# BurryChen/lv_slam

Measured on AMD Instinct MI355X. Metric: NDT registrations/sec (64k-pt Velodyne pairs), higher is better.
Workload: dtype f32 terms, f64 accumulation

## Files before the change

### include/mi355_ndt.h

```cpp
#ifndef MI355_NDT_H_
#define MI355_NDT_H_

#include <stddef.h>
#include <stdint.h>

#ifdef __cplusplus
extern "C" {
#endif

#define MI355NDT_OK               0
#define MI355NDT_ERR_BAD_HANDLE  (-1)
#define MI355NDT_ERR_BAD_ARG     (-2)
#define MI355NDT_ERR_HIP         (-3)
#define MI355NDT_ERR_GRID        (-4)
#define MI355NDT_ERR_NO_DEVICE   (-5)
#define MI355NDT_ERR_UNSUPPORTED (-6)
#define MI355NDT_WARN_TOLERANCE_ARITH 1
#define MI355NDT_TOLERANCE_MIN_HITS   4096
#define MI355NDT_ERR_STATE       (-7)

enum mi355ndt_neighbor { MI355NDT_KDTREE = 0, MI355NDT_DIRECT26 = 1, MI355NDT_DIRECT7 = 2, MI355NDT_DIRECT1 = 3 };
enum mi355ndt_variant { MI355NDT_VARIANT_OMP = 0 , MI355NDT_VARIANT_PCA = 1  };

typedef struct mi355ndt_params {
  float  resolution;
  double step_size;
  double outlier_ratio;
  double trans_epsilon;
  int    max_iterations;
  int    neighbor_mode;
  int    variant;
  int    min_points_per_voxel;
  double min_covar_eigvalue_mult;
} mi355ndt_params;

typedef struct mi355ndt_result {
  float     final_colmajor[16];
  double    trans_probability;
  double    score;
  int       iterations;
  int       converged;
  int       sweeps;
  int       status;
  long long hits_last;
} mi355ndt_result;

typedef struct mi355ndt_voxel {
  int32_t idx;
  int32_t n;
  double  mean[3];
  float   icov[9];
  int32_t weight;
} mi355ndt_voxel;

typedef struct mi355ndt_profile {
  double    sweep_ms;
  long long sweep_launches;
  double    sweep_alg_bytes;
  long long sweep_hits;
  long long sweep_points;
  double    build_ms;
  long long build_launches;
  double    build_alg_bytes;
  double    update_ms;
  long long update_launches;
  long long async_fallbacks;
  long long stream_launches;
  long long stream_carried;
  long long stream_redone;
  long long cloud_uploads;
  long long cloud_upload_bytes;
  long long cloud_transfers;
  long long cloud_promotions;
  long long stream_reserved_slots;
  long long stream_launch_slots;
} mi355ndt_profile;

typedef struct mi355ndt_handle mi355ndt_handle;

const char* mi355ndt_version(void);
int mi355ndt_device_count(void);
int mi355ndt_host_numa_node(int device);

int mi355ndt_default_params(mi355ndt_params* p);

int mi355ndt_create(const mi355ndt_params* params, int device, mi355ndt_handle** out);
int mi355ndt_destroy(mi355ndt_handle* h);

int mi355ndt_set_params(mi355ndt_handle* h, const mi355ndt_params* params);
int mi355ndt_get_params(const mi355ndt_handle* h, mi355ndt_params* out);

int mi355ndt_set_stream(mi355ndt_handle* h, void* hip_stream);
const char* mi355ndt_last_error(const mi355ndt_handle* h);


int mi355ndt_set_target(mi355ndt_handle* h, const void* pts, size_t n, size_t stride_bytes);
int mi355ndt_set_source(mi355ndt_handle* h, const void* pts, size_t n, size_t stride_bytes);
int mi355ndt_promote_source_to_target(mi355ndt_handle* h);
int mi355ndt_align(mi355ndt_handle* h, const float guess_colmajor[16], mi355ndt_result* out);
int mi355ndt_get_aligned(mi355ndt_handle* h, void* out_pts, size_t stride_bytes);

int mi355ndt_get_incremental(mi355ndt_handle* h, int pair, float transformation_colmajor[16], float previous_colmajor[16]);

int mi355ndt_get_fitness_score(mi355ndt_handle* h, double max_range, double* score, long long* n_inliers);
int mi355ndt_fitness_score_T(mi355ndt_handle* h, const float T_colmajor[16], double max_range, double* score, long long* n_inliers);

int mi355ndt_calculate_score(mi355ndt_handle* h, const void* pts, size_t n, size_t stride_bytes, double* score);

int mi355ndt_convert_transform(const double x[6], float out_colmajor[16]);

enum mi355ndt_option {
  MI355NDT_OPT_F32_SUM_ORDER = 1,
  MI355NDT_OPT_ASYNC_ALIGN = 2,
  MI355NDT_OPT_DEBUG_ASYNC_ABORT = 3,
  MI355NDT_OPT_STREAM_THRESHOLD = 4,
  MI355NDT_OPT_STREAM_RESERVE = 5,
  MI355NDT_OPT_DEBUG_ASYNC_RINGS = 6,
  MI355NDT_OPT_ARITH = 7
};
int mi355ndt_set_option(mi355ndt_handle* h, int option, int value);
int mi355ndt_get_option(const mi355ndt_handle* h, int option, int* value);

int mi355ndt_derivatives(mi355ndt_handle* h, const double p[6], double* score, double g[6], double H[36], long long* hits);
int mi355ndt_compute_hessian(mi355ndt_handle* h, const double p[6], double H[36]);
int mi355ndt_derivatives_T(mi355ndt_handle* h, const float T_colmajor[16], const float Rj_rowmajor[9],
                           double* score, double g[6], double H[36], long long* hits);
int mi355ndt_get_grid(mi355ndt_handle* h, int pair, int min_b[3], int max_b[3], int div_b[3], int* n_voxels);
int mi355ndt_get_voxels(mi355ndt_handle* h, int pair, mi355ndt_voxel* out, size_t capacity);


int mi355ndt_batch_reserve(mi355ndt_handle* h, int n_pairs, size_t max_target_pts, size_t max_source_pts);
int mi355ndt_batch_set_target(mi355ndt_handle* h, int pair, const void* pts, size_t n, size_t stride_bytes);
int mi355ndt_batch_set_source(mi355ndt_handle* h, int pair, const void* pts, size_t n, size_t stride_bytes);
int mi355ndt_batch_set_clouds(mi355ndt_handle* h, int first_pair, int n, const void* const* targets, const size_t* target_counts,
                              const void* const* sources, const size_t* source_counts, size_t stride_bytes, int n_threads);
int mi355ndt_batch_bind_device(mi355ndt_handle* h, int n_pairs,
                               const float* d_targets, const int* target_counts, size_t target_pitch,
                               const float* d_sources, const int* source_counts, size_t source_pitch);
int mi355ndt_batch_build_targets(mi355ndt_handle* h);
int mi355ndt_batch_align(mi355ndt_handle* h, const float* guesses_colmajor, mi355ndt_result* out);
int mi355ndt_batch_size(const mi355ndt_handle* h);
int mi355ndt_batch_fitness_scores(mi355ndt_handle* h, const float* T_colmajor, double max_range, double* scores, long long* n_inliers);
int mi355ndt_batch_pose_records(mi355ndt_handle* h, int id_base, int id_stride, void* d_records, size_t capacity);

int mi355ndt_stream_begin(mi355ndt_handle* h, int n_contexts , int max_pairs, size_t max_target_pts, size_t max_source_pts);
int mi355ndt_stream_submit(mi355ndt_handle* h, int n_pairs, const float* d_targets, const int* target_counts, size_t target_pitch,
                           const float* d_sources, const int* source_counts, size_t source_pitch, const float* guesses_colmajor,
                           long long* batch_id);
int mi355ndt_stream_submit_host(mi355ndt_handle* h, int n_pairs, const void* const* targets, const size_t* target_counts, const void* const* sources,
                                const size_t* source_counts, size_t stride_bytes, const float* guesses_colmajor, int n_threads, long long* batch_id);
int mi355ndt_stream_collect(mi355ndt_handle* h, long long batch_id, mi355ndt_result* out);
int mi355ndt_stream_pose_records(mi355ndt_handle* h, void* d_records, size_t capacity, int id_base, int id_stride);
int mi355ndt_pack_pose_records(const mi355ndt_result* results, int n, int id_base, int id_stride, void* records, size_t capacity);
int mi355ndt_stream_end(mi355ndt_handle* h);

int mi355ndt_set_latency_mode(mi355ndt_handle* h, int on);

typedef struct mi355ndt_seq_params {
  double keyframe_delta_trans;
  double keyframe_delta_angle;
  double keyframe_delta_time;
} mi355ndt_seq_params;

typedef struct mi355ndt_seq_frame {
  double odom_colmajor[16];
  float  tf_s2k_colmajor[16];
  double trans_probability;
  double dx, da, dt;
  int    key_id;
  int    new_keyframe;
  int    iterations, converged;
// ... 31 lines not shown
```

### lv_slam_amd/csrc/mi355_ndt.hip

```cpp
#include <hip/hip_runtime.h>

#include <cstdio>
#include <cstdlib>
#include <cstddef>
#include <cstring>
#include <string>
#include <vector>
#include <algorithm>
#include <cmath>
#include <mutex>
#include <atomic>
#include <thread>
#include <sched.h>
#include <fstream>
#include <chrono>

#include "mi355_ndt.h"
#include "ndt_math.hpp"
#include "ndt_types.hpp"
#include "ndt_build.hpp"
#include "ndt_segsort.hpp"
#include "ndt_sweep.hpp"
#include "ndt_update.hpp"
#include "ndt_hessian.hpp"
// ... 16 lines not shown
  int device = 0;
  hipStream_t stream = nullptr;
  bool own_stream = true;
  mi355ndt_params prm;
  std::string err;

  int n_pairs = 0, cap_pairs = 0;
  size_t tgt_pitch = 0, src_pitch = 0;
  size_t own_tgt_pitch = 0, own_src_pitch = 0;
  int own_tgt_pairs = 0, own_src_pairs = 0;
  float *d_tgt_own = nullptr, *d_src_own = nullptr;
  const float *d_tgt = nullptr, *d_src = nullptr;
  int *d_tgt_cnt = nullptr, *d_src_cnt = nullptr;
  std::vector<int> h_tgt_cnt, h_src_cnt;
  std::vector<int> up_tgt_cnt, up_src_cnt;
  bool targets_built = false, have_target = false, have_source = false;
  bool aligned_once = false;
  bool icov64_built = false;
  bool cent_built = false;
  float grid_resolution = 0.f;

  unsigned* d_minmax = nullptr;
  GridDesc* d_grid = nullptr;
  unsigned *d_nwords = nullptr, *d_word_off = nullptr;
  unsigned *d_keys_a = nullptr, *d_keys_b = nullptr;
  unsigned *d_vals_a = nullptr, *d_vals_b = nullptr;
  size_t keys_cap = 0;
  BitWord* d_words = nullptr; size_t words_cap = 0;
  VoxelRec* d_recs = nullptr; int *d_vox_idx = nullptr, *d_vox_n = nullptr;
  unsigned* d_seg_start = nullptr; double* d_sums = nullptr;
  unsigned *d_heads = nullptr, *d_head_cnt = nullptr; size_t heads_cap = 0, head_cnt_cap = 0;
  float* d_cent = nullptr; double* d_icov64 = nullptr; size_t icov64_cap = 0;
  int* d_kdw = nullptr; size_t kdw_cap = 0; bool kdw_built = false;
  float4* d_sorted = nullptr; size_t sorted_cap = 0; bool leaf_sorted = false;
  unsigned* d_rs_hist = nullptr; unsigned* d_rs_offs = nullptr; size_t rs_cap = 0;
  unsigned *d_cstart = nullptr, *d_cend = nullptr; size_t cell_cap = 0; bool cells_ready = false; int last_cb = 0;
  double* d_fit = nullptr; size_t fit_cap = 0;
  BitWord* d_fwords = nullptr; size_t fwords_cap = 0; unsigned* d_fruns = nullptr; size_t fruns_cap = 0; bool fit_index_ready = false;
  int* d_fit_items = nullptr; size_t fit_items_cap = 0; float* d_fit_T = nullptr; size_t fit_T_cap = 0;
  float *d_pf_in = nullptr, *d_pf_out = nullptr; unsigned char* d_pf_keep = nullptr; unsigned *d_pf_keys = nullptr, *d_pf_vals = nullptr;
  int *d_pf_flag = nullptr, *d_pf_pos = nullptr, *d_pf_mm = nullptr; PfGrid* d_pf_grid = nullptr; void* d_pf_tmp = nullptr;
  size_t pf_cap = 0, pf_tmp_bytes = 0; int pf_count = 0; size_t pf_pitch = 0;
  float last_final[16] = {1,0,0,0, 0,1,0,0, 0,0,1,0, 0,0,0,1};
  size_t recs_per_pair = 0, recs_cap = 0;
  unsigned* h_pin_u = nullptr;

  PairState* d_state = nullptr;
  double* d_partials = nullptr; size_t partials_cap = 0;
  int chunks_per_pair = 0;
  int rows_per_pair = 0, pts_per_chunk = CHUNK_PTS;
  int items_per_pair = 0;
  bool async_force = false;
  bool async_align = true;
  int* d_ring = nullptr; size_t ring_cap_total = 0; unsigned* d_arrived = nullptr; size_t arrived_cap = 0; AsyncCtl* d_actl = nullptr;
  AsyncCtl* h_pin_actl = nullptr;
  AsyncTab* d_atab = nullptr;
  unsigned debug_abort_pos = 0xFFFFFFFFu;
  unsigned debug_ring_mask = 0xFFu;
  int arith = 0;
  VoxelRecF* d_recs_fast = nullptr; size_t recs_fast_cap = 0; bool recs_fast_built = false;
  int f32_sum_order = 0;
  double gauss_last[3] = {0, 0, 0};
  float* d_score_pts = nullptr; size_t score_pts_cap = 0; double* d_score_part = nullptr; size_t score_part_cap = 0;
  bool latency_mode = false;
  bool seq_running = false;
  int fine_it = 0;
  int fine_tiles = 2;
  int* d_grid_of = nullptr; size_t grid_of_cap = 0;
  const int* d_grid_of_use = nullptr;
  SeqState* d_seq = nullptr; mi355ndt_seq_frame* d_seq_out = nullptr; double* d_stamps = nullptr; size_t seq_cap = 0;
  volatile int* h_seq_flags = nullptr; int* d_seq_flags = nullptr;
  float* d_guess = nullptr;
  float* h_pin_guess = nullptr;
  mi355ndt_result* d_results = nullptr;
  int* d_active = nullptr;
  int* d_active_list = nullptr;
  SweepCtl* d_ctl = nullptr;
  int ctl_idx = 0;
  int n_cu = 256;
  int dyn_shift = -1;
  int* h_pin_active = nullptr;
  hipEvent_t ev_burst[2] = {nullptr, nullptr};
  unsigned long long* d_hits = nullptr;
  float* d_hook = nullptr;
  float* d_aligned = nullptr; size_t aligned_cap = 0;
  float* h_pin_aligned = nullptr; size_t pin_aligned_cap = 0;
  struct UpSlot { float* h = nullptr; float* d = nullptr; size_t cap = 0; hipEvent_t ev = nullptr; bool used = false, filling = false; };
  static constexpr int UP_SLOTS = 12;
  UpSlot up[UP_SLOTS];
  int up_next = 0;
  static constexpr int UP_STREAMS = 4;
  hipStream_t copy_stream[UP_STREAMS] = {nullptr, nullptr, nullptr, nullptr};
  hipEvent_t ev_uploads[UP_STREAMS] = {nullptr, nullptr, nullptr, nullptr}, ev_compute = nullptr;
  bool uploads_pending = false;
  std::mutex up_mtx;

  bool async_build = false;
  int plan_cb = 0; size_t plan_words = 0;
  unsigned* d_bstat = nullptr;
  bool counts_preloaded = false;
  bool build_stamped = false;
  bool word_off_cleared = false;
  size_t last_total_words = 0;

  struct StreamCtx {
    mi355ndt_handle* e = nullptr;
// ... 161 lines not shown
  std::ifstream f("/sys/devices/system/node/node" + std::to_string(node) + "/cpulist");
  std::string txt;
  if (!f || !std::getline(f, txt)) return false;
  bool any = false;
  size_t pos = 0;
  while (pos < txt.size()) {
    size_t comma = txt.find(',', pos);
    std::string part = txt.substr(pos, comma == std::string::npos ? std::string::npos : comma - pos);
    size_t dash = part.find('-');
    int lo = atoi(part.c_str()), hi = dash == std::string::npos ? lo : atoi(part.c_str() + dash + 1);
    for (int c = lo; c <= hi && c < CPU_SETSIZE; c++) { CPU_SET(c, set); any = true; }
    if (comma == std::string::npos) break;
    pos = comma + 1;
  }
  return any;
}

int mi355ndt_default_params(mi355ndt_params* p) {
  if (!p) return MI355NDT_ERR_BAD_ARG;
  p->resolution = 1.0f;
  p->step_size = 0.1;
  p->outlier_ratio = 0.55;
  p->trans_epsilon = 0.1;
  p->max_iterations = 35;
  p->neighbor_mode = MI355NDT_DIRECT7;
  p->variant = MI355NDT_VARIANT_OMP;
  p->min_points_per_voxel = 6;
  p->min_covar_eigvalue_mult = 0.01;
  return MI355NDT_OK;
}

int mi355ndt_destroy(mi355ndt_handle* h);

int mi355ndt_create(const mi355ndt_params* params, int device, mi355ndt_handle** out) {
  if (!out) return MI355NDT_ERR_BAD_ARG;
  *out = nullptr;
  int n = 0;
  if (hipGetDeviceCount(&n) != hipSuccess || n <= 0) return MI355NDT_ERR_NO_DEVICE;
  if (device < 0 || device >= n) return MI355NDT_ERR_BAD_ARG;
  mi355ndt_params p;
  mi355ndt_default_params(&p);
  if (params) p = *params;
  int rc = check_params(p);
  if (rc) return rc;
  mi355ndt_handle* h = new mi355ndt_handle();
  h->device = device;
  h->prm = p;
  gauss_constants3(0.55, 1.0f, h->gauss_last);
  { hipDeviceProp_t pr; if (hipGetDeviceProperties(&pr, device) == hipSuccess && pr.multiProcessorCount > 0) h->n_cu = pr.multiProcessorCount; }
  if (const char* e = std::getenv("MI355NDT_LEAF_SORTED")) h->leaf_sorted = std::atoi(e) != 0;
  if (const char* e = std::getenv("MI355NDT_FINE_TILES")) { const int v = std::atoi(e); if (v == 1 || v == 2) h->fine_tiles = v; }
  if (const char* e = std::getenv("MI355NDT_ARITH")) h->arith = std::atoi(e) == 1 ? 1 : 0;
  if (const char* e = std::getenv("MI355NDT_ASYNC")) { h->async_align = std::atoi(e) != 0; h->async_force = std::atoi(e) == 2; }
  if (const char* e = std::getenv("MI355NDT_SWEEP_DYN_SHIFT")) { const int v = std::atoi(e); if (v >= 0 && v <= 30) h->dyn_shift = v; }
  if (hipSetDevice(device) != hipSuccess || hipStreamCreateWithFlags(&h->stream, hipStreamNonBlocking) != hipSuccess) {
    delete h;
    return MI355NDT_ERR_HIP;
  }
  if (hipHostMalloc((void**)&h->h_pin_u, 4 * sizeof(unsigned)) != hipSuccess ||
      hipHostMalloc((void**)&h->h_pin_active, 128 * sizeof(int)) != hipSuccess ||
      hipMalloc((void**)&h->d_active, 128 * sizeof(int)) != hipSuccess ||
      hipMalloc((void**)&h->d_ctl, 2 * sizeof(SweepCtl)) != hipSuccess ||
      hipMalloc((void**)&h->d_hits, sizeof(unsigned long long)) != hipSuccess ||
      hipMalloc((void**)&h->d_hook, 64 * sizeof(double)) != hipSuccess ||
      hipEventCreateWithFlags(&h->ev_compute, hipEventDisableTiming) != hipSuccess ||
      hipEventCreateWithFlags(&h->ev_burst[0], hipEventDisableTiming) != hipSuccess ||
      hipEventCreateWithFlags(&h->ev_burst[1], hipEventDisableTiming) != hipSuccess) {
    mi355ndt_destroy(h);
    return MI355NDT_ERR_HIP;
  }
  for (int i = 0; i < mi355ndt_handle::UP_STREAMS; i++)
    if (hipStreamCreateWithFlags(&h->copy_stream[i], hipStreamNonBlocking) != hipSuccess ||
        hipEventCreateWithFlags(&h->ev_uploads[i], hipEventDisableTiming) != hipSuccess) { mi355ndt_destroy(h); return MI355NDT_ERR_HIP; }
  *out = h;
  return MI355NDT_OK;
}

int mi355ndt_stream_end(mi355ndt_handle* h);
int mi355ndt_destroy(mi355ndt_handle* h) {
  if (!h) return MI355NDT_ERR_BAD_HANDLE;
  (void)hipSetDevice(h->device);
  (void)hipStreamSynchronize(h->stream);
  if (h->stream_on) (void)mi355ndt_stream_end(h);
  void* ptrs[] = {h->d_tgt_own, h->d_src_own, h->d_tgt_cnt, h->d_src_cnt, h->d_grid, h->d_nwords, h->d_word_off,
                  h->d_keys_a, h->d_keys_b, h->d_vals_a, h->d_vals_b, h->d_words, h->d_recs, h->d_vox_idx, h->d_vox_n,
                  h->d_state, h->d_partials, h->d_guess, h->d_results, h->d_active, h->d_hook, h->d_aligned, h->d_hits, h->d_seg_start, h->d_heads, h->d_head_cnt, h->d_sums,
                  h->d_cent, h->d_icov64, h->d_kdw, h->d_rs_hist, h->d_rs_offs, h->d_active_list, h->d_ctl, h->d_cstart, h->d_cend, h->d_fit, h->d_fwords, h->d_fruns, h->d_fit_items, h->d_fit_T, h->d_pf_in, h->d_pf_out, h->d_pf_keep, h->d_pf_keys,
                  h->d_pf_vals, h->d_pf_flag, h->d_pf_pos, h->d_pf_mm, h->d_pf_grid, h->d_pf_tmp, h->d_score_pts, h->d_score_part,
                  h->d_ring, h->d_arrived, h->d_actl, h->d_atab, h->d_sorted, h->d_recs_fast};
  for (void* p : ptrs) if (p) (void)hipFree(p);
  for (void* p : {(void*)h->d_grid_of, (void*)h->d_seq, (void*)h->d_seq_out, (void*)h->d_stamps}) if (p) (void)hipFree(p);
  if (h->h_seq_flags) (void)hipHostFree((void*)h->h_seq_flags);
  for (hipStream_t cs : h->copy_stream) if (cs) (void)hipStreamSynchronize(cs);
  for (auto& u : h->up) { if (u.h) (void)hipHostFree(u.h); if (u.d) (void)hipFree(u.d); if (u.ev) (void)hipEventDestroy(u.ev); }
  if (h->h_pin_aligned) (void)hipHostFree(h->h_pin_aligned);
  for (hipEvent_t e : h->ev_uploads) if (e) (void)hipEventDestroy(e);
  if (h->ev_compute) (void)hipEventDestroy(h->ev_compute);
  for (hipStream_t cs : h->copy_stream) if (cs) (void)hipStreamDestroy(cs);
  if (h->h_pin_actl) (void)hipHostFree(h->h_pin_actl);
  if (h->h_pin_u) (void)hipHostFree(h->h_pin_u);
  if (h->h_pin_active) (void)hipHostFree(h->h_pin_active);
  if (h->h_pin_guess) (void)hipHostFree(h->h_pin_guess);
  for (hipEvent_t e : h->ev_burst) if (e) (void)hipEventDestroy(e);
  for (hipEvent_t e : h->ev_pool) (void)hipEventDestroy(e);
  for (auto* v : {&h->ev_sweep, &h->ev_update, &h->ev_build})
    for (auto& e : *v) { if (!e.first_shared) (void)hipEventDestroy(e.first); (void)hipEventDestroy(e.second); }
  if (h->own_stream && h->stream) (void)hipStreamDestroy(h->stream);
  delete h;
  return MI355NDT_OK;
}

int mi355ndt_get_params(const mi355ndt_handle* h, mi355ndt_params* out) {
  if (!h) return MI355NDT_ERR_BAD_HANDLE;
  if (!out) return MI355NDT_ERR_BAD_ARG;
  *out = h->prm;
  return MI355NDT_OK;
// ... 296 lines not shown
  if (h->ev_last_fresh && h->ev_last) {
    v.push_back({h->ev_last, nullptr, true});
    h->ev_last_fresh = false;
    return hipSuccess;
  }
  hipEvent_t a;
  hipError_t e = ev_take(h, &a); if (e != hipSuccess) return e;
  v.push_back({a, nullptr, false});
  return hipEventRecord(a, h->stream);
}
static hipError_t ev_end(mi355ndt_handle* h, std::vector<mi355ndt_handle::EvSpan>& v) {
  hipEvent_t b;
  hipError_t e = ev_take(h, &b); if (e != hipSuccess) return e;
  v.back().second = b;
  h->ev_last = b;
  h->ev_last_fresh = true;
  return hipEventRecord(b, h->stream);
}
static void ev_collect(mi355ndt_handle* h, std::vector<mi355ndt_handle::EvSpan>& v, double& ms, long long& n) {
  for (auto& e : v) {
    float t = 0;
    if (e.second && hipEventElapsedTime(&t, e.first, e.second) == hipSuccess) { ms += t; n++; }
    if (!e.first_shared) h->ev_pool.push_back(e.first);
    if (e.second) h->ev_pool.push_back(e.second);
  }
  v.clear();
  h->ev_last_fresh = false;
}
int mi355ndt_profile_enable(mi355ndt_handle* h, int on) {
  if (!h) return MI355NDT_ERR_BAD_HANDLE;
  h->prof = on != 0;
  if (h->stream_on) for (int c = 0; c < h->s_nctx; c++) if (h->sctx[c].e) { h->sctx[c].e->ev_pool_target = 128; (void)mi355ndt_profile_enable(h->sctx[c].e, on); }
  if (h->prof) {
    HIPCHK(h, hipSetDevice(h->device));
    while (h->ev_pool.size() < h->ev_pool_target) {
      hipEvent_t e;
      HIPCHK(h, hipEventCreate(&e));
      h->ev_pool.push_back(e);
    }
  }
  return MI355NDT_OK;
}
int mi355ndt_profile_reset(mi355ndt_handle* h) {
  if (!h) return MI355NDT_ERR_BAD_HANDLE;
  (void)hipSetDevice(h->device);
  (void)hipStreamSynchronize(h->stream);
  double d; long long n;
  ev_collect(h, h->ev_sweep, d, n); ev_collect(h, h->ev_update, d, n); ev_collect(h, h->ev_build, d, n);
  if (h->stream_on) for (int c = 0; c < h->s_nctx; c++) if (mi355ndt_handle* e = h->sctx[c].e) {
    ev_collect(e, e->ev_sweep, d, n); ev_collect(e, e->ev_update, d, n); ev_collect(e, e->ev_build, d, n);
    e->P = mi355ndt_profile{};
  }
  h->P = mi355ndt_profile{};
  (void)hipMemsetAsync(h->d_hits, 0, sizeof(unsigned long long), h->stream);
  (void)hipStreamSynchronize(h->stream);
  return MI355NDT_OK;
}
int mi355ndt_profile_get(mi355ndt_handle* h, mi355ndt_profile* out) {
  if (!h) return MI355NDT_ERR_BAD_HANDLE;
  if (!out) return MI355NDT_ERR_BAD_ARG;
  HIPCHK(h, hipSetDevice(h->device));
  HIPCHK(h, hipStreamSynchronize(h->stream));
  ev_collect(h, h->ev_sweep, h->P.sweep_ms, h->P.sweep_launches);
  ev_collect(h, h->ev_update, h->P.update_ms, h->P.update_launches);
  ev_collect(h, h->ev_build, h->P.build_ms, h->P.build_launches);
  if (h->stream_on) for (int c = 0; c < h->s_nctx; c++) if (mi355ndt_handle* e = h->sctx[c].e) {
    ev_collect(e, e->ev_sweep, h->P.sweep_ms, h->P.sweep_launches);
    ev_collect(e, e->ev_update, h->P.update_ms, h->P.update_launches);
    ev_collect(e, e->ev_build, h->P.build_ms, h->P.build_launches);
    h->P.build_alg_bytes += e->P.build_alg_bytes; e->P.build_alg_bytes = 0;
    { std::lock_guard<std::mutex> lk(e->up_mtx);
      h->P.cloud_uploads += e->P.cloud_uploads; e->P.cloud_uploads = 0; h->P.cloud_upload_bytes += e->P.cloud_upload_bytes; e->P.cloud_upload_bytes = 0;
      h->P.cloud_transfers += e->P.cloud_transfers; e->P.cloud_transfers = 0; }
  }
  unsigned long long hh = 0;
  HIPCHK(h, hipMemcpy(&hh, h->d_hits, sizeof hh, hipMemcpyDeviceToHost));
  *out = h->P;
  if (h->stream_on) { out->stream_reserved_slots = h->s_reserve_wg; out->stream_launch_slots = h->s_launch_slots; }
  out->sweep_hits += (long long)hh;
  out->sweep_alg_bytes += 64.0 * (double)hh;
  return MI355NDT_OK;
}

static int build_targets_impl(mi355ndt_handle* h);
int mi355ndt_batch_build_targets(mi355ndt_handle* h) {
  if (!h) return MI355NDT_ERR_BAD_HANDLE;
  NOT_IN_STREAM(h);
  const int rc = build_targets_impl(h);
  if (rc != MI355NDT_OK && h->ev_compute) (void)compute_enqueued(h);
  return rc;
}
static int build_targets_impl(mi355ndt_handle* h) {
  if (h->n_pairs <= 0 || !h->d_tgt) return MI355NDT_ERR_STATE;
  HIPCHK(h, hipSetDevice(h->device));
  { int rcu = uploads_before_compute(h); if (rcu) return rcu; }
  const int B = h->n_pairs;
  const size_t pitch = h->tgt_pitch;
  const size_t total = (size_t)B * pitch;
  hipStream_t s = h->stream;
  if (h->async_build && h->counts_preloaded) {
    h->up_tgt_cnt.clear();
  } else if (h->up_tgt_cnt.size() != (size_t)B || !std::equal(h->up_tgt_cnt.begin(), h->up_tgt_cnt.end(), h->h_tgt_cnt.begin())) {
    HIPCHK(h, hipMemcpyAsync(h->d_tgt_cnt, h->h_tgt_cnt.data(), B * sizeof(int), hipMemcpyHostToDevice, s));
    HIPCHK(h, hipStreamSynchronize(s));
    h->up_tgt_cnt.assign(h->h_tgt_cnt.begin(), h->h_tgt_cnt.begin() + B);
  }

  if (total > h->keys_cap) {
    size_t c1 = h->keys_cap, c2 = h->keys_cap, c3 = h->keys_cap, c4 = h->keys_cap;
    HIPCHK(h, grow(h->d_keys_a, c1, total)); HIPCHK(h, grow(h->d_keys_b, c2, total));
    HIPCHK(h, grow(h->d_vals_a, c3, total)); HIPCHK(h, grow(h->d_vals_b, c4, total));
    h->keys_cap = total;
  }
  const int minpts = h->prm.min_points_per_voxel;
  const size_t rpp = pitch / (size_t)minpts + 1;
  if (rpp > ((size_t)1 << ID_BITS)) { h->err = "target too large: voxel ids would not fit the sweep's queue entries"; return MI355NDT_ERR_BAD_ARG; }
  if ((size_t)B * rpp > h->recs_cap || rpp != h->recs_per_pair) {
    size_t need = (size_t)B * rpp, c1 = 0, c2 = 0, c3 = 0, c4 = 0, c5 = 0;
    if (h->d_recs) { HIPCHK(h, hipFree(h->d_recs)); h->d_recs = nullptr; }
    if (h->d_vox_idx) { HIPCHK(h, hipFree(h->d_vox_idx)); h->d_vox_idx = nullptr; }
    if (h->d_vox_n) { HIPCHK(h, hipFree(h->d_vox_n)); h->d_vox_n = nullptr; }
    if (h->d_seg_start) { HIPCHK(h, hipFree(h->d_seg_start)); h->d_seg_start = nullptr; }
    if (h->d_sums) { HIPCHK(h, hipFree(h->d_sums)); h->d_sums = nullptr; }
    if (h->d_cent) { HIPCHK(h, hipFree(h->d_cent)); h->d_cent = nullptr; }
    HIPCHK(h, grow(h->d_recs, c1, need)); HIPCHK(h, grow(h->d_vox_idx, c2, need)); HIPCHK(h, grow(h->d_vox_n, c3, need));
    HIPCHK(h, grow(h->d_seg_start, c4, need)); HIPCHK(h, grow(h->d_sums, c5, need * 9));
    { size_t c6 = 0; HIPCHK(h, grow(h->d_cent, c6, need * 3)); }
    h->recs_cap = need; h->recs_per_pair = rpp;
  }
  h->ev_last_fresh = false;
  const bool build_events = h->prof && !(h->build_stamped && h->async_build);
  if (build_events) HIPCHK(h, ev_begin(h, h->ev_build));
  const int gx = (int)((pitch + 255) / 256);
// ... 275 lines not shown
  unsigned long long* stamp_end = nullptr;
  int claim_items = 1;
  int reserve_wg = 0;
  hipEvent_t ev_prepared = nullptr;
};
#define NDT_CTX_ARGS(i) L.tab.c[i].src, L.tab.c[i].pitch, L.tab.c[i].st, L.tab.c[i].gd, L.tab.c[i].words, L.tab.c[i].recs, L.tab.c[i].partials, L.tab.c[i].src_cnt, \
                        L.tab.c[i].arrived, L.tab.c[i].cent
template <bool PCA, int K, int ORD>
static int launch_async_t(mi355ndt_handle* h, const SweepConst& sc, const AsyncLaunch& L) {
  auto kern = k_align_async<PCA, K, ORD>;
  static std::atomic<int> per_cu_of_device[64];
  int per_cu = per_cu_of_device[h->device & 63].load(std::memory_order_relaxed);
  if (per_cu == 0) {
    if (hipOccupancyMaxActiveBlocksPerMultiprocessor(&per_cu, kern, SWEEP_THREADS, 0) != hipSuccess) { (void)hipGetLastError(); return MI355NDT_ERR_UNSUPPORTED; }
    per_cu_of_device[h->device & 63].store(per_cu, std::memory_order_relaxed);
  }
  const int wpe = sweep_wpe(PCA, K, ORD == 2);
  if (per_cu < wpe || h->n_cu * wpe < 8) return MI355NDT_ERR_UNSUPPORTED;
  dim3 grid((unsigned)std::max(8, h->n_cu * wpe - L.reserve_wg));
  kern<<<grid, SWEEP_THREADS, 0, h->stream>>>(L.tab_dev, L.items_per_pair, L.ring, L.ring_cap, L.ctl, sc, h->prof ? h->d_hits : nullptr,
                                             h->prm.step_size, h->prm.trans_epsilon, h->prm.max_iterations, L.stop_thresh, L.debug_abort_pos, L.debug_ring_mask, L.claim_items,
                                             NDT_CTX_ARGS(0), NDT_CTX_ARGS(1), NDT_CTX_ARGS(2), NDT_CTX_ARGS(3));
  return MI355NDT_OK;
}
template <bool PCA, int K>
static int launch_async_o(mi355ndt_handle* h, const SweepConst& sc, const AsyncLaunch& L) {
  if constexpr (K == 1 || K == 7) { if (sweep_ord(h, sc) == 2) return launch_async_t<PCA, K, 2>(h, sc, L); }
  return h->f32_sum_order == 1 ? launch_async_t<PCA, K, 1>(h, sc, L) : launch_async_t<PCA, K, 0>(h, sc, L);
}
static int launch_async(mi355ndt_handle* h, const SweepConst& sc, const AsyncLaunch& L) {
  hipStream_t s = h->stream;
  {
    const size_t n = std::max(std::max(std::max((size_t)8 * L.ring_cap, (size_t)L.n_new * ASYNC_ARR_STRIDE), sizeof(AsyncCtl) / sizeof(unsigned)), (size_t)L.pose_cap);
    k_async_prepare<<<(unsigned)((n + 255) / 256), 256, 0, s>>>(L.tab, L.tab_dev, L.new_ci, L.n_new, L.st_new, L.guess_new, L.src_cnt_new, L.gd_new, L.arrived_new,
                                                               L.active_list, L.sweep_ctl, L.ring, L.ring_cap, L.ctl, L.prev, L.done_new, L.pose_new, L.pose_cap, L.stamp_end);
    if (L.ev_prepared) HIPCHK(h, hipEventRecord(L.ev_prepared, s));
  }
  if (h->prof) HIPCHK(h, ev_begin(h, h->ev_sweep));
  int rc;
  if (sc.pca) rc = sc.K == 1 ? launch_async_o<true, 1>(h, sc, L) : sc.K == 7 ? launch_async_o<true, 7>(h, sc, L) : launch_async_o<true, 26>(h, sc, L);
  else rc = sc.K == 1 ? launch_async_o<false, 1>(h, sc, L) : sc.K == 7 ? launch_async_o<false, 7>(h, sc, L)
          : sc.K == 26 ? launch_async_o<false, 26>(h, sc, L) : launch_async_o<false, 27>(h, sc, L);
  if (h->prof) HIPCHK(h, ev_end(h, h->ev_sweep));
  return rc;
}
static int async_ring_cap(const mi355ndt_handle* h, long long pairs) {
  const long long cap = (pairs * ((long long)h->prm.max_iterations + 4) + 7) / 8 + 1;
  return cap > (1LL << 26) ? 0 : (int)cap;
}
static void fill_async_ctx(const mi355ndt_handle* e, AsyncCtx& c) {
  SweepConst sc;
  make_sweep_const(e, sc);
  c.src = e->d_src; c.pitch = e->src_pitch; c.st = e->d_state; c.gd = e->d_grid; c.words = e->d_words; c.recs = sweep_recs(e, sc); c.cent = e->d_cent;
  c.partials = e->d_partials; c.src_cnt = e->d_src_cnt; c.arrived = e->d_arrived; c.results = e->d_results; c.n_done = nullptr; c.must_finish = 1; c.pose = nullptr; c.pose_base = 0; c.pose_stride = 0; c.pad_ = 0;
}
extern "C" {
static int align_async(mi355ndt_handle* h, const SweepConst& sc, int B, mi355ndt_result* out) {
  hipStream_t s = h->stream;
  const int ring_cap = async_ring_cap(h, B);
  if (ring_cap == 0) return MI355NDT_ERR_UNSUPPORTED;
  if (grow(h->d_ring, h->ring_cap_total, (size_t)8 * ring_cap) != hipSuccess) { (void)hipGetLastError(); return MI355NDT_ERR_UNSUPPORTED; }
  HIPCHK(h, grow(h->d_arrived, h->arrived_cap, (size_t)B * ASYNC_ARR_STRIDE));
  if (!h->d_actl) HIPCHK(h, hipMalloc((void**)&h->d_actl, sizeof(AsyncCtl)));
  if (!h->d_atab) HIPCHK(h, hipMalloc((void**)&h->d_atab, sizeof(AsyncTab)));
  if (!h->h_pin_actl) HIPCHK(h, hipHostMalloc((void**)&h->h_pin_actl, sizeof(AsyncCtl)));
  AsyncLaunch L;
  memset(&L.tab, 0, sizeof L.tab);
  fill_async_ctx(h, L.tab.c[0]);
  L.new_ci = 0; L.n_new = B;
  L.st_new = h->d_state; L.guess_new = h->d_guess; L.src_cnt_new = h->d_src_cnt; L.gd_new = h->d_grid; L.arrived_new = h->d_arrived;
  L.active_list = h->d_active_list; L.sweep_ctl = h->d_ctl;
  L.tab_dev = h->d_atab; L.ring = h->d_ring; L.ring_cap = ring_cap; L.ctl = h->d_actl; L.prev = nullptr;
  L.items_per_pair = h->items_per_pair; L.stop_thresh = 0; L.debug_abort_pos = h->debug_abort_pos; L.debug_ring_mask = h->debug_ring_mask;
  int rc = launch_async(h, sc, L);
  if (rc) return rc;
  HIPCHK(h, hipMemcpyAsync(h->h_pin_actl, h->d_actl, 8 * sizeof(unsigned), hipMemcpyDeviceToHost, s));
  HIPCHK(h, hipMemcpyAsync(out, h->d_results, (size_t)B * sizeof(mi355ndt_result), hipMemcpyDeviceToHost, s));
  HIPCHK(h, hipStreamSynchronize(s));
  HIPCHK(h, hipGetLastError());
  if (h->h_pin_actl->abort_ || h->h_pin_actl->fin != (unsigned)B) {
    h->P.async_fallbacks++;
    return MI355NDT_ERR_UNSUPPORTED;
  }
  if (h->prof) {
    for (int b = 0; b < B; b++) {
      h->P.sweep_alg_bytes += (double)out[b].sweeps * h->h_src_cnt[b] * (12.0 + 4.0 * sc.K);
      h->P.sweep_points += (long long)out[b].sweeps * h->h_src_cnt[b];
    }
  }
  return MI355NDT_OK;
}

static int batch_align_impl(mi355ndt_handle* h, const float* guesses, mi355ndt_result* out) {
  if (!guesses || !out) return MI355NDT_ERR_BAD_ARG;
  if (h->n_pairs <= 0 || !h->d_tgt || !h->d_src) return MI355NDT_ERR_STATE;
  HIPCHK(h, hipSetDevice(h->device));
  { int rcu = uploads_before_compute(h); if (rcu) return rcu; }
  const bool mt_live = mt_is_live(h->prm);
  const bool pca_kd = h->prm.neighbor_mode == MI355NDT_KDTREE && h->prm.variant == MI355NDT_VARIANT_PCA;
  if (!h->targets_built || (mt_live && !h->icov64_built) || (pca_kd && !h->kdw_built) || (fast_served(h) && !h->recs_fast_built)) { int rc = mi355ndt_batch_build_targets(h); if (rc) return rc; }
  int rc = prep_align_ws(h);
  if (rc) return rc;
  const int B = h->n_pairs;
  hipStream_t s = h->stream;
  SweepConst sc;
  make_sweep_const(h, sc);
  gauss_constants3(h->prm.outlier_ratio, h->prm.resolution, h->gauss_last);
// ... 543 lines not shown
  int rc = upload_cloud(h, h->d_score_pts, pitch, 0, pts, n, stride);
  if (rc) return rc;
  rc = uploads_before_compute(h);
  if (rc) return rc;
  SweepConst sc;
  make_sweep_const(h, sc);
  hipStream_t s = h->stream;
  k_calc_score<<<blocks, SCORE_THREADS, 0, s>>>(h->d_score_pts, pitch, (int)n, h->d_grid, h->d_words, h->d_recs, h->d_icov64, h->d_cent,
                                                h->gauss_last[0], h->gauss_last[1], h->gauss_last[2], sc.kd_r2, sc.leaf_pow2, sc.inv_leaf, h->d_score_part);
  std::vector<double> part((size_t)blocks);
  HIPCHK(h, hipMemcpyAsync(part.data(), h->d_score_part, part.size() * sizeof(double), hipMemcpyDeviceToHost, s));
  HIPCHK(h, hipStreamSynchronize(s));
  HIPCHK(h, hipGetLastError());
  double sum = 0;
  for (int b = 0; b < blocks; b++) sum += part[(size_t)b];
  *score = sum / (double)n;
  return compute_enqueued(h);
}

static void aa_matrix(float angle, int axis, float R[9]) {
  const float ax[3] = {axis == 0 ? 1.f : 0.f, axis == 1 ? 1.f : 0.f, axis == 2 ? 1.f : 0.f};
  const float sn = sinf(angle), c = cosf(angle);
  const float sa[3] = {sn * ax[0], sn * ax[1], sn * ax[2]};
  const float c1[3] = {(1.f - c) * ax[0], (1.f - c) * ax[1], (1.f - c) * ax[2]};
  float tmp = c1[0] * ax[1];
  R[0 * 3 + 1] = tmp - sa[2]; R[1 * 3 + 0] = tmp + sa[2];
  tmp = c1[0] * ax[2];
  R[0 * 3 + 2] = tmp + sa[1]; R[2 * 3 + 0] = tmp - sa[1];
  tmp = c1[1] * ax[2];
  R[1 * 3 + 2] = tmp - sa[0]; R[2 * 3 + 1] = tmp + sa[0];
  for (int a = 0; a < 3; a++) R[a * 3 + a] = c1[a] * ax[a] + c;
}
static void mul33(const float A[9], const float B[9], float C[9]) {
  for (int r = 0; r < 3; r++)
    for (int c = 0; c < 3; c++) C[r * 3 + c] = A[r * 3 + 0] * B[0 * 3 + c] + (A[r * 3 + 1] * B[1 * 3 + c] + A[r * 3 + 2] * B[2 * 3 + c]);
}
int mi355ndt_convert_transform(const double x[6], float out[16]) {
  if (!x || !out) return MI355NDT_ERR_BAD_ARG;
  float Rx[9], Ry[9], Rz[9], A[9], L[9];
  aa_matrix((float)x[3], 0, Rx); aa_matrix((float)x[4], 1, Ry); aa_matrix((float)x[5], 2, Rz);
  mul33(Rx, Ry, A);
  mul33(A, Rz, L);
  for (int r = 0; r < 3; r++) {
    for (int c = 0; c < 3; c++) out[c * 4 + r] = L[r * 3 + c];
    out[12 + r] = (float)x[r];
    out[r * 4 + 3] = 0.f;
  }
  out[15] = 1.f;
  return MI355NDT_OK;
}

int mi355ndt_set_option(mi355ndt_handle* h, int option, int value) {
  if (!h) return MI355NDT_ERR_BAD_HANDLE;
  if (h->stream_on && (option == MI355NDT_OPT_F32_SUM_ORDER || option == MI355NDT_OPT_ARITH || option == MI355NDT_OPT_ASYNC_ALIGN)) NOT_IN_STREAM(h);
  if (option == MI355NDT_OPT_F32_SUM_ORDER) {
    if (value != 0 && value != 1) return MI355NDT_ERR_BAD_ARG;
    h->f32_sum_order = value;
    return MI355NDT_OK;
  }
  if (option == MI355NDT_OPT_ARITH) {
    if (value != 0 && value != 1) return MI355NDT_ERR_BAD_ARG;
    h->arith = value;
    return MI355NDT_OK;
  }
  if (option == MI355NDT_OPT_ASYNC_ALIGN) {
    if (value < 0 || value > 2) return MI355NDT_ERR_BAD_ARG;
    h->async_align = value != 0;
    h->async_force = value == 2;
    return MI355NDT_OK;
  }
  if (option == MI355NDT_OPT_DEBUG_ASYNC_ABORT) {
    h->debug_abort_pos = value < 0 ? 0xFFFFFFFFu : (unsigned)value;
    return MI355NDT_OK;
  }
  if (option == MI355NDT_OPT_DEBUG_ASYNC_RINGS) {
    if ((value & 0xFF) == 0) return MI355NDT_ERR_BAD_ARG;
    h->debug_ring_mask = (unsigned)value & 0xFFu;
    return MI355NDT_OK;
  }
  if (option == MI355NDT_OPT_STREAM_THRESHOLD) {
    if (value < -1 || value > ASYNC_MAX_CARRY) return MI355NDT_ERR_BAD_ARG;
    h->s_thresh_opt = value;
    return MI355NDT_OK;
  }
  if (option == MI355NDT_OPT_STREAM_RESERVE) {
    if (value < -1 || value > 4096) return MI355NDT_ERR_BAD_ARG;
    h->s_reserve_opt = value;
    return MI355NDT_OK;
  }
  return MI355NDT_ERR_BAD_ARG;
}
int mi355ndt_get_option(const mi355ndt_handle* h, int option, int* value) {
  if (!h) return MI355NDT_ERR_BAD_HANDLE;
  if (!value) return MI355NDT_ERR_BAD_ARG;
  if (option == MI355NDT_OPT_F32_SUM_ORDER) { *value = h->f32_sum_order; return MI355NDT_OK; }
  if (option == MI355NDT_OPT_ARITH) { *value = h->arith; return MI355NDT_OK; }
  if (option == MI355NDT_OPT_ASYNC_ALIGN) { *value = h->async_force ? 2 : (h->async_align ? 1 : 0); return MI355NDT_OK; }
  if (option == MI355NDT_OPT_DEBUG_ASYNC_ABORT) { *value = h->debug_abort_pos == 0xFFFFFFFFu ? -1 : (int)h->debug_abort_pos; return MI355NDT_OK; }
  if (option == MI355NDT_OPT_DEBUG_ASYNC_RINGS) { *value = (int)h->debug_ring_mask; return MI355NDT_OK; }
  if (option == MI355NDT_OPT_STREAM_THRESHOLD) { *value = h->s_thresh_opt; return MI355NDT_OK; }
  if (option == MI355NDT_OPT_STREAM_RESERVE) { *value = h->s_reserve_opt; return MI355NDT_OK; }
  return MI355NDT_ERR_BAD_ARG;
}

int mi355ndt_prefilter(mi355ndt_handle* h, const void* pts, size_t n, size_t stride,
                       int use_distance_filter, double distance_near, double distance_far, float downsample_resolution,
                       void* out_pts, size_t out_capacity, size_t out_stride, size_t* n_out) {
  if (!h) return MI355NDT_ERR_BAD_HANDLE;
  if ((!pts && n) || (n && stride < 12) || n >= (1u << 30) || !n_out || (out_pts && out_stride < 12)) return MI355NDT_ERR_BAD_ARG;
  if (std::isnan(downsample_resolution)) return MI355NDT_ERR_BAD_ARG;
  *n_out = 0;
  h->pf_count = 0;
  if (n == 0) return MI355NDT_OK;
  HIPCHK(h, hipSetDevice(h->device));
  hipStream_t s = h->stream;
  const size_t pitch = (n + 63) & ~(size_t)63;
  if (pitch > h->pf_cap) {
    HIPCHK(h, hipStreamSynchronize(s));
    void** ps[] = {(void**)&h->d_pf_in, (void**)&h->d_pf_out, (void**)&h->d_pf_keep, (void**)&h->d_pf_keys, (void**)&h->d_pf_vals,
                   (void**)&h->d_pf_flag, (void**)&h->d_pf_pos};
    const size_t bytes[] = {3 * pitch * 4, 3 * pitch * 4, pitch, 2 * pitch * 4, 2 * pitch * 4, pitch * 4, pitch * 4};
    for (int i = 0; i < 7; i++) { if (*ps[i]) { HIPCHK(h, hipFree(*ps[i])); *ps[i] = nullptr; } HIPCHK(h, hipMalloc(ps[i], bytes[i])); }
    if (!h->d_pf_mm) HIPCHK(h, hipMalloc((void**)&h->d_pf_mm, 6 * sizeof(int)));
    if (!h->d_pf_grid) HIPCHK(h, hipMalloc((void**)&h->d_pf_grid, sizeof(PfGrid)));
    h->pf_cap = pitch;
  }
  h->pf_pitch = pitch;
  int rc = upload_cloud(h, h->d_pf_in, pitch, 0, pts, n, stride);
  if (rc) return rc;
  rc = uploads_before_compute(h);
  if (rc) return rc;
  const int gx = (int)((pitch + 255) / 256);
  unsigned *ka = h->d_pf_keys, *kb = h->d_pf_keys + pitch, *va = h->d_pf_vals, *vb = h->d_pf_vals + pitch;
  const int pf_tiles = (int)((pitch + RS_TILE - 1) / RS_TILE);
  const int pf_chunks = (int)((pitch + PF_SCAN_CHUNK - 1) / PF_SCAN_CHUNK);
  {
    const size_t need = (size_t)pf_tiles << RS_MAX_BITS;
    if (need > h->rs_cap) {
      size_t c1 = 0, c2 = 0;
      if (h->d_rs_hist) { HIPCHK(h, hipFree(h->d_rs_hist)); h->d_rs_hist = nullptr; }
      if (h->d_rs_offs) { HIPCHK(h, hipFree(h->d_rs_offs)); h->d_rs_offs = nullptr; }
      HIPCHK(h, grow(h->d_rs_hist, c1, need)); HIPCHK(h, grow(h->d_rs_offs, c2, need));
      h->rs_cap = need;
    }
    const size_t nb = (size_t)pf_chunks * sizeof(unsigned);
    if (nb > h->pf_tmp_bytes) {
      if (h->d_pf_tmp) { HIPCHK(h, hipFree(h->d_pf_tmp)); h->d_pf_tmp = nullptr; }
      HIPCHK(h, hipMalloc(&h->d_pf_tmp, nb));
      h->pf_tmp_bytes = nb;
    }
// ... 136 lines not shown
}

int mi355ndt_stream_begin(mi355ndt_handle* h, int n_contexts, int max_pairs, size_t max_tgt, size_t max_src) {
  if (!h) return MI355NDT_ERR_BAD_HANDLE;
  if (n_contexts < 2 || n_contexts > ASYNC_MAX_CTX || max_pairs < 1 || max_pairs > MAX_PAIRS || max_pairs >= (1 << ASYNC_CTX_SHIFT) ||
      max_tgt == 0 || max_src == 0 || max_tgt >= (1u << 31) || max_src >= (1u << 31)) return MI355NDT_ERR_BAD_ARG;
  if (h->stream_on) return MI355NDT_ERR_STATE;
  HIPCHK(h, hipSetDevice(h->device));
  HIPCHK(h, hipStreamSynchronize(h->stream));
  h->s_nctx = n_contexts; h->s_max_pairs = max_pairs; h->s_max_tgt = max_tgt; h->s_max_src = max_src;
  h->s_items = std::max(1, (int)((max_src + CHUNK_PTS - 1) / CHUNK_PTS)) * QUARTERS;
  h->s_sync_only = !stream_async_ok(h);
  h->s_next_id = 0; h->s_launches = 0; h->s_counted = 0; h->s_drop_carry = true; h->s_recovered_upto = -1;
  h->s_plan_cb = 0; h->s_plan_words = 0;
  h->targets_built = false; h->grid_resolution = 0.f; h->recs_fast_built = false;
  SweepConst sc;
  make_sweep_const(h, sc);
  {
    const int iu = h->s_items / (sc.K == 1 ? ((want_fast(h, sc) && FAST_D1_POINT) ? FAST_CLAIM1 : 2) : sc.K == 7 ? 2 : 1);
    const int waves = h->n_cu * sweep_wpe(sc.pca != 0, sc.K, want_fast(h, sc)) * WAVES;
    int t = h->s_thresh_opt >= 0 ? h->s_thresh_opt : 4 * ((waves + iu - 1) / std::max(1, iu));
    if (const char* e = std::getenv("MI355NDT_STREAM_THRESH")) t = std::atoi(e);
    h->s_thresh = std::max(0, std::min(t, ASYNC_MAX_CARRY));
  }
  {
    const bool small_batch = (unsigned long long)max_pairs * (unsigned long long)max_tgt <= 768ull * 65536ull;
    int r = sc.K == 1 ? (max_tgt <= 98304 ? 128 : 96) : ((sc.K == 7 && small_batch) ? (sc.pca ? 32 : 64) : 0);
    if (const char* e = std::getenv("MI355NDT_STREAM_RESERVE")) r = std::atoi(e);
    if (h->s_reserve_opt >= 0) r = h->s_reserve_opt;
    r = std::max(0, std::min(r, h->n_cu * sweep_wpe(sc.pca != 0, sc.K, want_fast(h, sc)) / 2)) & ~7;
    if (n_contexts < 3) r = 0;
    h->s_reserve_wg = r;
    h->s_launch_slots = std::max(8, h->n_cu * sweep_wpe(sc.pca != 0, sc.K, want_fast(h, sc)) - r);
  }
  h->s_ring_cap = async_ring_cap(h, (long long)max_pairs + ASYNC_MAX_CARRY);
  if (h->s_ring_cap == 0) h->s_sync_only = true;
  auto fail = [&](int rc) { (void)stream_free(h); return rc; };
  if (hipMalloc((void**)&h->d_sstat, ASYNC_MAX_CTX * sizeof(CtxStat)) != hipSuccess ||
      hipMemsetAsync(h->d_sstat, 0, ASYNC_MAX_CTX * sizeof(CtxStat), h->stream) != hipSuccess) return fail(MI355NDT_ERR_HIP);
  for (int c = 0; c < n_contexts; c++) {
    mi355ndt_handle::StreamCtx& S = h->sctx[c];
    int rc = mi355ndt_create(&h->prm, h->device, &S.e);
    if (rc) return fail(rc);
    mi355ndt_handle* e = S.e;
    if (h->s_reserve_wg > 0 && !h->s_build_stream) {
      if (hipStreamCreateWithFlags(&h->s_build_stream, hipStreamNonBlocking) != hipSuccess) return fail(MI355NDT_ERR_HIP);
      for (auto& ev : h->s_ev_built) if (hipEventCreateWithFlags(&ev, hipEventDisableTiming) != hipSuccess) return fail(MI355NDT_ERR_HIP);
      for (auto& ev : h->s_ev_launched) if (hipEventCreateWithFlags(&ev, hipEventDisableTiming) != hipSuccess) return fail(MI355NDT_ERR_HIP);
      for (auto& ev : h->s_ev_prepared) if (hipEventCreateWithFlags(&ev, hipEventDisableTiming) != hipSuccess) return fail(MI355NDT_ERR_HIP);
      if (const char* pf = std::getenv("MI355NDT_STREAM_PREP_FIRST")) h->s_prep_first = std::atoi(pf) != 0;
    }
    rc = mi355ndt_set_stream(e, h->s_reserve_wg > 0 ? h->s_build_stream : h->stream);
    if (rc) return fail(rc);
    e->f32_sum_order = h->f32_sum_order; e->arith = h->arith; e->async_align = h->async_align; e->dyn_shift = h->dyn_shift;
    e->async_build = true;
    e->ev_pool_target = 128;
    rc = ensure_pair_arrays(e, max_pairs);
    if (rc) { h->err = e->err; return fail(rc); }
    S.in_bytes = (size_t)max_pairs * (2 * sizeof(int) + 16 * sizeof(float));
    if (hipMalloc((void**)&S.d_in, S.in_bytes) != hipSuccess || hipHostMalloc((void**)&S.h_in, S.in_bytes, hipHostMallocMapped) != hipSuccess ||
        hipHostGetDevicePointer((void**)&S.h_in_dev, S.h_in, 0) != hipSuccess ||
        hipHostMalloc((void**)&S.h_res, (size_t)max_pairs * sizeof(mi355ndt_result), hipHostMallocMapped | hipHostMallocCoherent) != hipSuccess ||
        hipHostGetDevicePointer((void**)&S.d_res_map, S.h_res, 0) != hipSuccess) { h->err = "stream_begin: allocation failed"; return fail(MI355NDT_ERR_HIP); }
    S.own_tgt_cnt = e->d_tgt_cnt; S.own_src_cnt = e->d_src_cnt; S.own_guess = e->d_guess;
    e->d_tgt_cnt = S.d_in; e->d_src_cnt = S.d_in + max_pairs; e->d_guess = (float*)(S.d_in + 2 * (size_t)max_pairs);
    e->d_bstat = reinterpret_cast<unsigned*>(h->d_sstat + c);
    size_t need = (size_t)max_pairs * h->s_items * NACC;
    if (grow(e->d_partials, e->partials_cap, need) != hipSuccess || grow(e->d_arrived, e->arrived_cap, (size_t)max_pairs * ASYNC_ARR_STRIDE) != hipSuccess)
      { h->err = "stream_begin: allocation failed"; return fail(MI355NDT_ERR_HIP); }
    if (h->prof) (void)mi355ndt_profile_enable(e, 1);
  }
  if (hipMalloc((void**)&h->d_sctl, 2 * sizeof(AsyncCtl)) != hipSuccess || hipMemsetAsync(h->d_sctl, 0, 2 * sizeof(AsyncCtl), h->stream) != hipSuccess ||
      hipHostMalloc((void**)&h->h_sstatus, mi355ndt_handle::S_EV * sizeof(StreamStatus), hipHostMallocMapped | hipHostMallocCoherent) != hipSuccess ||
      hipHostGetDevicePointer((void**)&h->d_sstatus, (void*)h->h_sstatus, 0) != hipSuccess) return fail(MI355NDT_ERR_HIP);
  memset((void*)h->h_sstatus, 0, mi355ndt_handle::S_EV * sizeof(StreamStatus));
  if (!h->d_atab && hipMalloc((void**)&h->d_atab, sizeof(AsyncTab)) != hipSuccess) return fail(MI355NDT_ERR_HIP);
  if (!h->s_sync_only && hipMalloc((void**)&h->d_sring, (size_t)8 * h->s_ring_cap * sizeof(int)) != hipSuccess) { (void)hipGetLastError(); h->s_sync_only = true; }
  if (h->s_build_stream) HIPCHK(h, hipStreamSynchronize(h->s_build_stream));
  HIPCHK(h, hipStreamSynchronize(h->stream));
  (void)max_tgt;
  h->stream_on = true;
  return MI355NDT_OK;
}

static int stream_launch(mi355ndt_handle* h, int new_ci, int n_new) {
  hipStream_t s = h->stream;
  SweepConst sc;
  make_sweep_const(h, sc);
  AsyncLaunch L;
  memset(&L.tab, 0, sizeof L.tab);
  const bool flush = new_ci < 0;
  for (int c = 0; c < h->s_nctx; c++) {
    mi355ndt_handle* e = h->sctx[c].e;
    if (!e->d_src) continue;
    fill_async_ctx(e, L.tab.c[c]);
    L.tab.c[c].results = h->sctx[c].d_res_map;
    L.tab.c[c].n_done = &h->d_sstat[c].done;
    L.tab.c[c].pose = h->sctx[c].busy ? h->sctx[c].d_pose : nullptr; L.tab.c[c].pose_base = h->sctx[c].pose_base; L.tab.c[c].pose_stride = h->sctx[c].pose_stride;
    const int ahead = (h->s_reserve_wg > 0 || h->s_nctx >= 3) ? 2 : 1;
    bool mf = flush;
    for (int a = 1; a <= ahead; a++) mf = mf || c == (new_ci + a) % h->s_nctx;
    L.tab.c[c].must_finish = mf ? 1 : 0;
  }
  const long long j = h->s_launches;
  L.new_ci = flush ? 0 : new_ci; L.n_new = flush ? 0 : n_new;
  if (!flush) {
    mi355ndt_handle* e = h->sctx[new_ci].e;
// ... 395 lines not shown
```

### lv_slam_amd/csrc/ndt_async.hpp

```cpp
#pragma once
#include "ndt_types.hpp"
#include "ndt_math.hpp"
#include "ndt_sweep.hpp"
#include "ndt_update.hpp"

#define ASYNC_POS_STRIDE 32
#define ASYNC_ARR_STRIDE 16
#define ASYNC_MAX_CTX    4
#define ASYNC_MAX_CARRY  128
#define ASYNC_CTX_SHIFT  24

struct AsyncCtx {
  const float* src; size_t pitch;
  PairState* st; const GridDesc* gd; const BitWord* words; const VoxelRec* recs; const float* cent;
  double* partials; const int* src_cnt; unsigned* arrived; mi355ndt_result* results;
  unsigned* n_done;
  int must_finish;
  int pose_base; PoseRecord* pose; int pose_stride, pad_;
};
struct AsyncTab { AsyncCtx c[ASYNC_MAX_CTX]; };
#define NDT_GP(T) __attribute__((address_space(1))) T*
struct AsyncCtxG {
  NDT_GP(const float) src; size_t pitch;
  NDT_GP(PairState) st; NDT_GP(const GridDesc) gd; NDT_GP(const BitWord) words; NDT_GP(const VoxelRec) recs; NDT_GP(const float) cent;
  NDT_GP(double) partials; NDT_GP(const int) src_cnt; NDT_GP(unsigned) arrived; NDT_GP(mi355ndt_result) results;
  NDT_GP(unsigned) n_done;
  int must_finish;
  int pose_base; NDT_GP(PoseRecord) pose; int pose_stride, pad_;
};
static_assert(sizeof(AsyncCtxG) == sizeof(AsyncCtx) && offsetof(AsyncCtxG, pose) == offsetof(AsyncCtx, pose) && offsetof(AsyncCtxG, n_done) == offsetof(AsyncCtx, n_done),
              "AsyncCtxG mirrors AsyncCtx");
__device__ __forceinline__ AsyncCtx async_ctx_load(const AsyncTab* __restrict__ tab, const int ci) {
  const AsyncCtxG& g = reinterpret_cast<const AsyncCtxG*>(tab->c)[ci];
  AsyncCtx c;
  c.src = (const float*)g.src; c.pitch = g.pitch; c.st = (PairState*)g.st; c.gd = (const GridDesc*)g.gd; c.words = (const BitWord*)g.words;
  c.recs = (const VoxelRec*)g.recs; c.cent = (const float*)g.cent; c.partials = (double*)g.partials; c.src_cnt = (const int*)g.src_cnt;
  c.arrived = (unsigned*)g.arrived; c.results = (mi355ndt_result*)g.results; c.n_done = (unsigned*)g.n_done; c.must_finish = g.must_finish;
  c.pose_base = g.pose_base; c.pose = (PoseRecord*)g.pose; c.pose_stride = g.pose_stride; c.pad_ = 0;
  return c;
}
struct CtxStat { unsigned done, total_words, max_cells, plan_exceeded; };
struct StreamStatus { unsigned fin, abort_, n_live, susp; CtxStat ctx[ASYNC_MAX_CTX]; unsigned seq; unsigned pad0_;
                      unsigned long long build_t0, build_t1;
                      unsigned pad_[6]; };
static_assert(sizeof(StreamStatus) == 128, "one status slot is 128 bytes");

struct AsyncCtl {
  unsigned pub;
  unsigned fin;
  unsigned abort_;
  unsigned n_live;
  unsigned susp;
  unsigned pad_[27];
  unsigned pos[8 * ASYNC_POS_STRIDE];
  unsigned carry[ASYNC_MAX_CARRY];
};

#ifndef ASYNC_CLAIM
#define ASYNC_CLAIM(K) ((K) == 1 ? 2 : 1)
#endif
#ifndef ASYNC_HELP_RINGS
#define ASYNC_HELP_RINGS 1
#endif
#define ASYNC_HELP_AFTER 64u
#define ASYNC_SPIN_LIMIT (1u << 18)

NDT_KERNEL void k_async_prepare(const AsyncTab tab, AsyncTab* tab_dev, const int new_ci, const int n_new, PairState* st, const float* __restrict__ guess_cm,
                                const int* __restrict__ src_cnt, const GridDesc* __restrict__ gd, unsigned* arrived, int* active_list, SweepCtl* sweep_ctl ,
                                int* ring, const int ring_cap, AsyncCtl* ctl, const AsyncCtl* prev, unsigned* done_new ,
                                PoseRecord* pose_new , const int pose_cap, unsigned long long* stamp ) {
  const size_t i = (size_t)blockIdx.x * blockDim.x + threadIdx.x;
  if (i == 0 && stamp) *stamp = (unsigned long long)wall_clock64();
  const unsigned nc = prev ? min(prev->susp, (unsigned)ASYNC_MAX_CARRY) : 0u;
  const unsigned n_live = nc + (unsigned)n_new;
  if (i < (size_t)8 * ring_cap) {
    const size_t g = (i % (size_t)ring_cap) * 8 + i / (size_t)ring_cap;
    int w = -1;
    if (g < nc) w = (int)prev->carry[g];
    else if (g < n_live) w = (new_ci << ASYNC_CTX_SHIFT) | (int)(g - nc);
    ring[i] = w;
  }
  if (i < (size_t)n_new * ASYNC_ARR_STRIDE) arrived[i] = 0u;
  if (i < offsetof(AsyncCtl, carry) / sizeof(unsigned)) reinterpret_cast<unsigned*>(ctl)[i] = (i == 0 || i == 3) ? n_live : 0u;
  if (sweep_ctl && i < 2 * sizeof(SweepCtl) / sizeof(int)) reinterpret_cast<int*>(sweep_ctl)[i] = i == 0 ? n_new : 0;
  if (i == 0 && done_new && n_new > 0) *done_new = 0u;
  if (pose_new && i < (size_t)pose_cap) {
    PoseRecord r;
    memset(&r, 0, sizeof r);
    r.pair_id = -1;
    pose_new[i] = r;
  }
// ... 25 lines not shown
  gu64* sg = (gu64*)reinterpret_cast<unsigned long long*>(&st[b]);
  unsigned long long* sl = reinterpret_cast<unsigned long long*>(&Ssh);
  for (int i = lane; i < NW; i += 64) sl[i] = __hip_atomic_load(sg + i, RLX_AGENT);
  if (lane == 0) sol[6] = 0.0;
  const int nchunks = (n_pts + CHUNK_PTS - 1) / CHUNK_PTS;
  double aw0 = 0.0, aw1 = 0.0, aw2 = 0.0, aw3 = 0.0;
  if (lane < NACC) {
    const gu64* P = (const gu64*)reinterpret_cast<const unsigned long long*>(partials + (size_t)b * rows_per_pair * NACC + lane);
    auto ldq = [&](int c, int k) -> double { return __longlong_as_double((long long)__hip_atomic_load(P + ((size_t)c * 4 + k) * NACC, RLX_AGENT)); };
    auto addw = [&](int g, double gs) { const int w = g & 3; if (w == 0) aw0 += gs; else if (w == 1) aw1 += gs; else if (w == 2) aw2 += gs; else aw3 += gs; };
#pragma unroll 1
    for (int c0 = 0; c0 < nchunks; c0 += 16) {
      if (c0 + 16 <= nchunks) {
        double q[16][4];
#pragma unroll
        for (int u = 0; u < 16; u++)
#pragma unroll
          for (int k = 0; k < 4; k++) q[u][k] = ldq(c0 + u, k);
        double gs = 0.0;
#pragma unroll
        for (int u = 0; u < 8; u++) gs += ((q[u][0] + q[u][1]) + q[u][2]) + q[u][3];
        addw(c0 >> 3, gs);
        gs = 0.0;
#pragma unroll
        for (int u = 8; u < 16; u++) gs += ((q[u][0] + q[u][1]) + q[u][2]) + q[u][3];
        addw((c0 >> 3) + 1, gs);
      } else {
#pragma unroll 1
        for (int g0 = c0; g0 < nchunks; g0 += 8) {
          double gs = 0.0;
          if (g0 + 8 <= nchunks) {
            double q[8][4];
#pragma unroll
            for (int u = 0; u < 8; u++)
#pragma unroll
              for (int k = 0; k < 4; k++) q[u][k] = ldq(g0 + u, k);
#pragma unroll
            for (int u = 0; u < 8; u++) gs += ((q[u][0] + q[u][1]) + q[u][2]) + q[u][3];
          } else {
            for (int c = g0; c < nchunks; c++) {
              double r[4];
#pragma unroll
              for (int k = 0; k < 4; k++) r[k] = ldq(c, k);
              gs += ((r[0] + r[1]) + r[2]) + r[3];
            }
          }
          addw(g0 >> 3, gs);
        }
      }
    }
  }
  asm volatile("s_waitcnt lgkmcnt(0)" ::: "memory");
  __builtin_amdgcn_wave_barrier();
  if (lane < NACC) {
    double v = 0.0;
    v += aw0; v += aw1; v += aw2; v += aw3;
    if (lane == 0) Ssh.score = v;
    else if (lane < 7) Ssh.g[lane - 1] = v;
    else if (lane < 43) Ssh.H[lane - 7] = v;
    else { Ssh.hits = (long long)v; if (hits_total) atomicAdd(hits_total, (unsigned long long)v); }
  }
  asm volatile("s_waitcnt lgkmcnt(0)" ::: "memory");
  __builtin_amdgcn_wave_barrier();
  TL_STAMP(12);
  constexpr int RB0 = (int)(offsetof(PairState, reb_pn) / 8), RBT = (int)(offsetof(PairState, reb_tag) / 8);
  static_assert(RBT - RB0 == 14, "6 + 8 words of re-basing");
  const bool want_reb = Ssh.phase == PH_STEP;
  bool reb_ok = want_reb && Ssh.reb_tag == (long long)Ssh.sweeps;
  unsigned long long rbw = 0;
  if (reb_ok && lane < 14) rbw = __hip_atomic_load(sg + RB0 + lane, RLX_AGENT);
  newton_solve_side(Ssh, sol);
  asm volatile("s_waitcnt lgkmcnt(0)" ::: "memory");
  __builtin_amdgcn_wave_barrier();
  TL_STAMP(13);
  if (want_reb && !reb_ok) {
    unsigned spins = 0;
    while (!reb_ok && spins++ < (1u << 16)) {
      __builtin_amdgcn_s_sleep(2);
      long long tg = 0;
      if (lane == 0) tg = (long long)__hip_atomic_load(sg + RBT, RLX_AGENT);
      reb_ok = __shfl(tg, 0) == (long long)Ssh.sweeps;
    }
    if (reb_ok && lane < 14) rbw = __hip_atomic_load(sg + RB0 + lane, RLX_AGENT);
  }
  if (reb_ok && lane < 14) sl[RB0 + lane] = rbw;
  asm volatile("s_waitcnt lgkmcnt(0)" ::: "memory");
  __builtin_amdgcn_wave_barrier();
  const bool rebased = reb_ok;
  int rc = newton_update(Ssh, &results[b], step_max, eps, max_iterations, 0, sol, rebased);
  rc = __builtin_amdgcn_readfirstlane(rc);
  asm volatile("s_waitcnt lgkmcnt(0)" ::: "memory");
  __builtin_amdgcn_wave_barrier();
  TL_STAMP(14);
  for (int i = lane; i < NW; i += 64) __hip_atomic_store(sg + i, sl[i], RLX_AGENT);
  asm volatile("s_waitcnt vmcnt(0)" ::: "memory");
  if (lane == 0) {
    bool suspend = false;
    if (rc == NEWTON_SWEEP && stop_thresh > 0 && !C.must_finish)
      suspend = n_live - __hip_atomic_load((const gu32*)&ctl->fin, RLX_AGENT) <= (unsigned)stop_thresh;
    if (rc == NEWTON_SWEEP && !suspend) {
      const unsigned g = __hip_atomic_fetch_add((gu32*)&ctl->pub, 1u, RLX_AGENT);
      __hip_atomic_store((gu32*)reinterpret_cast<unsigned*>(ring + (size_t)(g & 7u) * ring_cap + (g >> 3)), (unsigned)tw, RLX_AGENT);
    } else if (rc == NEWTON_SWEEP) {
      const unsigned k = __hip_atomic_fetch_add((gu32*)&ctl->susp, 1u, RLX_AGENT);
      if (k < (unsigned)ASYNC_MAX_CARRY) __hip_atomic_store((gu32*)&ctl->carry[k], (unsigned)tw, RLX_AGENT);
      asm volatile("s_waitcnt vmcnt(0)" ::: "memory");
      __hip_atomic_fetch_add((gu32*)&ctl->fin, 1u, RLX_AGENT);
    } else {
      if (C.pose) {
        PoseRecord r;
        for (int a = 0; a < 16; a++) r.final_cm[a] = Ssh.final_cm[a];
        r.score = (float)Ssh.score; r.iterations = Ssh.it; r.converged = Ssh.converged; r.pair_id = C.pose_base + b * C.pose_stride;
        for (int a = 0; a < 4; a++) r.pad[a] = 0;
        C.pose[b] = r;
      }
      asm volatile("s_waitcnt vmcnt(0)" ::: "memory");
      if (C.n_done) __hip_atomic_fetch_add((gu32*)C.n_done, 1u, RLX_AGENT);
      __hip_atomic_fetch_add((gu32*)&ctl->fin, 1u, RLX_AGENT);
    }
  }
  TL_STAMP(9);
  if (rc == NEWTON_SWEEP) {
    constexpr int RBI = (int)(offsetof(PairState, reb_inc) / 8);
    double pn[6]; float inc[16];
    newton_rebase(Ssh.p, Ssh.dir, Ssh.a_t, pn, inc);
    if (lane == 0) {
      for (int a = 0; a < 6; a++) __hip_atomic_store(sg + RB0 + a, (unsigned long long)__double_as_longlong(pn[a]), RLX_AGENT);
      for (int a = 0; a < 8; a++)
        __hip_atomic_store(sg + RBI + a, (unsigned long long)__float_as_uint(inc[2 * a]) | ((unsigned long long)__float_as_uint(inc[2 * a + 1]) << 32), RLX_AGENT);
      asm volatile("s_waitcnt vmcnt(0)" ::: "memory");
      __hip_atomic_store(sg + RBT, (unsigned long long)(long long)Ssh.sweeps, RLX_AGENT);
    }
  }
  __builtin_amdgcn_s_setprio(0);
}

NDT_KERNEL void k_stream_inputs(const unsigned* __restrict__ host_in, unsigned* __restrict__ dev_in, const unsigned n_in, unsigned* __restrict__ clear, const unsigned n_clear,
                                unsigned long long* stamp) {
  if (threadIdx.x == 0 && stamp) *stamp = (unsigned long long)wall_clock64();
  for (unsigned i = threadIdx.x; i < n_in; i += blockDim.x) dev_in[i] = host_in[i];
  for (unsigned i = threadIdx.x; i < n_clear; i += blockDim.x) clear[i] = 0u;
}
// ... 61 lines not shown
        if (ASYNC_HELP_RINGS && spins >= ASYNC_HELP_AFTER && (spins & 3u) == 3u) {
          const unsigned y = ((unsigned)x + 1u + (spins >> 2) % 7u) & 7u;
          gu32* pos_y = (gu32*)&ctl->pos[y * ASYNC_POS_STRIDE];
          const unsigned q = __hip_atomic_load(pos_y, RLX_AGENT);
          const unsigned pubv = (unsigned)pf;
          const unsigned slots_y = pubv > y ? ((pubv - 1u - y) >> 3) + 1u : 0u;
          const unsigned tq = q / (unsigned)Iu;
          if (tq < slots_y && (int)tq < ring_cap) {
            unsigned expect = q;
            if (__hip_atomic_compare_exchange_strong(pos_y, &expect, q + 1u, __ATOMIC_RELAXED, __ATOMIC_RELAXED, __HIP_MEMORY_SCOPE_AGENT)) {
              const gu32* slot = (const gu32*)reinterpret_cast<const unsigned*>(ring + (size_t)y * ring_cap + tq);
              int ws = (int)__hip_atomic_load(slot, RLX_AGENT);
              unsigned lag = 0;
              while (ws < 0 && ++lag <= ASYNC_SPIN_LIMIT) { __builtin_amdgcn_s_sleep(2); ws = (int)__hip_atomic_load(slot, RLX_AGENT); }
              if (ws < 0) { give_up(); w = -2; break; }
              w = ws; sp = q; st = 1;
              break;
            }
          }
        }
        __builtin_amdgcn_s_sleep(32);
        if (t < ring_cap) w = (int)__hip_atomic_load(ringx + t, RLX_AGENT);
        if (++spins > ASYNC_SPIN_LIMIT) { give_up(); w = -2; break; }
      }
    }
    w = __builtin_amdgcn_readfirstlane(w);
    helped = __builtin_amdgcn_readfirstlane(st) != 0;
    if (helped) { held = true; held_pos = p; p = __builtin_amdgcn_readfirstlane(sp); }
    return w;
  };
  unsigned pos = 0;
  if (lane == 0) pos = __hip_atomic_fetch_add(pos_p, 1u, RLX_AGENT);
  pos = __builtin_amdgcn_readfirstlane(pos);
  int tw = -1;
  if (lane == 0 && (int)(pos / (unsigned)Iu) < ring_cap) tw = (int)__hip_atomic_load(ringx + pos / (unsigned)Iu, RLX_AGENT);
  tw = wait_ticket(pos, tw);
  if (tw < 0) return;
  unsigned pose_w = sweep_pose_words(NDT_CTX_SEL(st, tw >> ASYNC_CTX_SHIFT) + (tw & ((1 << ASYNC_CTX_SHIFT) - 1)));
#pragma unroll 1
  for (;;) {
    if (x == 0 && pos == debug_abort_pos) { if (lane == 0) give_up(); break; }
    const int rem = (int)(pos % (unsigned)Iu) * CLAIM;
    TL_STAMP(10);
    const int ci = tw >> ASYNC_CTX_SHIFT;
    AsyncCtx C = async_ctx_load(tab, ci);
    C.src = NDT_CTX_SEL(src, ci); C.pitch = NDT_CTX_SEL(pitch, ci); C.st = NDT_CTX_SEL(st, ci); C.gd = NDT_CTX_SEL(gd, ci); C.words = NDT_CTX_SEL(words, ci);
    C.recs = NDT_CTX_SEL(recs, ci); C.partials = NDT_CTX_SEL(partials, ci); C.src_cnt = NDT_CTX_SEL(src_cnt, ci); C.arrived = NDT_CTX_SEL(arrived, ci);
    C.cent = NDT_CTX_SEL(cent, ci);
    const int b = tw & ((1 << ASYNC_CTX_SHIFT) - 1);
    const int n_b = C.src_cnt[b];
#ifndef ASYNC_D1_PIPE
#define ASYNC_D1_PIPE 1
#endif
    if constexpr (K == 1 && ASYNC_D1_PIPE && ORD != 2) {
      sweep_rows_d1<PCA, ORD, CLAIM_D1>(b, rem, C.src, C.pitch, C.gd, C.words, C.recs, C.partials, I, sc, exp_tab, pose_w, n_b, b
#ifdef NDT_TIMELINE
                                     , tl, tl_last
#endif
                                     );
    } else if constexpr (K == 1 && ORD == 2 && FAST_D1_POINT) {
      float T[12], Rj[9];
#pragma unroll
      for (int a_ = 0; a_ < 12; a_++) T[a_] = __uint_as_float(__builtin_amdgcn_readlane(pose_w, a_));
#pragma unroll
      for (int a_ = 0; a_ < 9; a_++) Rj[a_] = __uint_as_float(__builtin_amdgcn_readlane(pose_w, 12 + a_));
      sweep_rows_d1p<PCA, CLAIM_D1, true>(b, rem, C.src, C.pitch, T, Rj, n_b, C.gd[b], C.words, C.recs, C.partials, I, sc
#ifdef NDT_TIMELINE
                                          , tl, tl_last
#endif
                                          );
    } else {
#pragma unroll 1
      for (int k = 0; k < CLAIM; k++)
        sweep_item<PCA, K, 8, false, ORD, true>(b, rem + k, C.src, C.pitch, C.st, C.gd, C.words, C.recs, C.partials, I, sc, C.cent, nullptr, exp_tab, pose_w, n_b, b
#ifdef NDT_TIMELINE
                                                , tl, tl_last
#endif
                                                );
    }
    unsigned npos = held_pos;
    if (lane == 0 && !held) npos = __hip_atomic_fetch_add(pos_p, 1u, RLX_AGENT);
    held = false;
    asm volatile("s_waitcnt vmcnt(0)" ::: "memory");
    npos = __builtin_amdgcn_readfirstlane(npos);
    const int tn = (int)(npos / (unsigned)Iu);
    unsigned old = 0;
    int ntw = -1;
    if (lane == 0) {
      old = __hip_atomic_fetch_add((gu32*)(C.arrived + (size_t)b * ASYNC_ARR_STRIDE), (unsigned)CLAIM, RLX_AGENT);
      if (tn < ring_cap) ntw = (int)__hip_atomic_load(ringx + tn, RLX_AGENT);
    }
    old = __builtin_amdgcn_readfirstlane(old);
    ntw = __builtin_amdgcn_readfirstlane(ntw);
    unsigned npose = 0;
    if (ntw >= 0) npose = sweep_pose_words(NDT_CTX_SEL(st, ntw >> ASYNC_CTX_SHIFT) + (ntw & ((1 << ASYNC_CTX_SHIFT) - 1)));
    TL_STAMP(8);
    if ((old + (unsigned)CLAIM) % (unsigned)I == 0u) {
      async_update(C, b, tw, n_b, I, Ssh[wv], sol[wv], ring, ring_cap, ctl, n_live, stop_thresh, hits_total, step_max, eps, max_iterations
#ifdef NDT_TIMELINE
                   , tl, tl_last
#endif
                   );
      TL_STAMP(15);
    }
    if (ntw < 0) {
      ntw = wait_ticket(npos, ntw);
      if (ntw < 0) break;
      npose = sweep_pose_words(NDT_CTX_SEL(st, ntw >> ASYNC_CTX_SHIFT) + (ntw & ((1 << ASYNC_CTX_SHIFT) - 1)));
    }
    tw = ntw; pos = npos; pose_w = npose;
  }
#ifdef NDT_TIMELINE
  if (lane == 0) for (int k = 0; k < 16; k++) atomicAdd(&g_tl[k], tl[k]);
#endif
}
```

### lv_slam_amd/csrc/ndt_sweep.hpp

```cpp
#pragma once
#include "ndt_types.hpp"
#include "ndt_math.hpp"
#include <type_traits>

struct NoHook { __device__ __forceinline__ void operator()() const {} };

template <int ORD>
__device__ __forceinline__ float sum3(float t0, float t1, float t2) { return ORD == 1 ? (t0 + t2) + t1 : (t0 + t1) + t2; }

template <bool PCA, typename Mid = NoHook, bool SAN = false, int ORD = 0>
__device__ __forceinline__ void eval_hit(const float u_in[3], const float r[3], const float C_in[9],
                                         const double d1, const float d2f, const double w, const bool ok_in, double acc[43],
                                         const double* __restrict__ exp_tab, Mid mid = Mid()) {
  float u[3] = {u_in[0], u_in[1], u_in[2]}, C[9];
#pragma unroll
  for (int a = 0; a < 9; a++) C[a] = C_in[a];
  float y[3];
#pragma unroll
  for (int j = 0; j < 3; j++) y[j] = sum3<ORD>(u[0] * C[j], u[1] * C[3 + j], u[2] * C[6 + j]);
  const float qf = sum3<ORD>(u[0] * y[0], u[1] * y[1], u[2] * y[2]);
  const float e0 = ndtm::exp_f32arg((-d2f * qf) * 0.5f, exp_tab);
  float s_inc = (float)(-d1 * (double)e0);
  const float e1 = d2f * e0;
  const bool ok = ok_in && !(e1 > 1.f || e1 < 0.f || e1 != e1);
  float e = (float)((double)e1 * d1);
  e = ok ? e : 0.f;
  s_inc = ok ? s_inc : 0.f;
  if (SAN) {
#pragma unroll
    for (int a = 0; a < 3; a++) { u[a] = ok ? u[a] : 0.f; y[a] = ok ? y[a] : 0.f; }
#pragma unroll
    for (int a = 0; a < 9; a++) C[a] = ok ? C[a] : 0.f;
  }
  float CJ[3][6];
#pragma unroll
  for (int a = 0; a < 3; a++) {
    CJ[a][0] = C[a * 3 + 0]; CJ[a][1] = C[a * 3 + 1]; CJ[a][2] = C[a * 3 + 2];
    CJ[a][3] = C[a * 3 + 1] * (-r[2]) + C[a * 3 + 2] * r[1];
    CJ[a][4] = C[a * 3 + 0] * r[2] + C[a * 3 + 2] * (-r[0]);
    CJ[a][5] = C[a * 3 + 0] * (-r[1]) + C[a * 3 + 1] * r[0];
  }
  float v[6];
#pragma unroll
  for (int k = 0; k < 6; k++) v[k] = sum3<ORD>(u[0] * CJ[0][k], u[1] * CJ[1][k], u[2] * CJ[2][k]);
#define NDT_ACC(slot, val) do { if (PCA) acc[slot] = fma(w, (double)(val), acc[slot]); else acc[slot] += (double)(val); } while (0)
  NDT_ACC(0, s_inc);
#pragma unroll
  for (int k = 0; k < 6; k++) NDT_ACC(1 + k, e * v[k]);
  float Z[3][3];
  Z[0][0] = y[1] * (-r[1]) + y[2] * (-r[2]);
  Z[1][0] = y[0] * r[1];
  Z[2][0] = y[0] * r[2];
  Z[0][1] = y[1] * r[0];
  Z[1][1] = y[0] * (-r[0]) + y[2] * (-r[2]);
  Z[2][1] = y[1] * r[2];
  Z[0][2] = y[2] * r[0];
  Z[1][2] = y[2] * r[1];
  Z[2][2] = y[0] * (-r[0]) + y[1] * (-r[1]);
  __builtin_amdgcn_sched_barrier(0);
  mid();
  __builtin_amdgcn_sched_barrier(0);
#pragma unroll
  for (int i = 0; i < 6; i++) {
#pragma unroll
    for (int j = 0; j < 6; j++) {
      float jcj;
      if (j < 3) jcj = CJ[j][i];
      else if (j == 3) jcj = (-r[2]) * CJ[1][i] + r[1] * CJ[2][i];
      else if (j == 4) jcj = r[2] * CJ[0][i] + (-r[0]) * CJ[2][i];
      else jcj = (-r[1]) * CJ[0][i] + r[0] * CJ[1][i];
      float t = ((-d2f) * v[i]) * v[j];
      if (i >= 3 && j >= 3) t = t + Z[i - 3][j - 3];
      const float h = e * (t + jcj);
      NDT_ACC(7 + i * 6 + j, h);
    }
  }
#undef NDT_ACC
}

#define NACC_F 37
__host__ __device__ constexpr int fsym(int i, int j) { return i <= j ? 7 + i * 6 - i * (i - 1) / 2 + (j - i) : 7 + j * 6 - j * (j - 1) / 2 + (i - j); }
#define FA_BASE 28
template <bool PCA, typename Mid = NoHook>
__device__ __forceinline__ void eval_hit_fast(const float u[3], const float r[3], const float c[6], const float d1f, const float d2f, const float kq,
                                              const float w, const bool ok_in, float a[NACC_F], Mid mid = Mid()) {
  const float c00 = c[0], c01 = c[1], c02 = c[2], c11 = c[3], c12 = c[4], c22 = c[5];
  float y[3];
  y[0] = fmaf(c02, u[2], fmaf(c01, u[1], c00 * u[0]));
  y[1] = fmaf(c12, u[2], fmaf(c11, u[1], c01 * u[0]));
  y[2] = fmaf(c22, u[2], fmaf(c12, u[1], c02 * u[0]));
  const float q = fmaf(u[2], y[2], fmaf(u[1], y[1], u[0] * y[0]));
  const float e0 = __builtin_amdgcn_exp2f(kq * q);
  const float e1 = d2f * e0;
  const bool ok = ok_in && !(e1 > 1.f || e1 < 0.f || e1 != e1);
  float e = e1 * d1f, s = -d1f * e0;
  if (PCA) { e *= w; s *= w; }
  e = ok ? e : 0.f;
  s = ok ? s : 0.f;
  a[0] += s;
  float v[6] = {y[0], y[1], y[2], fmaf(r[1], y[2], -(r[2] * y[1])), fmaf(r[2], y[0], -(r[0] * y[2])), fmaf(r[0], y[1], -(r[1] * y[0]))};
#pragma unroll
  for (int k = 0; k < 6; k++) a[1 + k] = fmaf(e, v[k], a[1 + k]);
  __builtin_amdgcn_sched_barrier(0);
  mid();
  __builtin_amdgcn_sched_barrier(0);
  const float C[3][3] = {{c00, c01, c02}, {c01, c11, c12}, {c02, c12, c22}};
  float M[3][3];
#pragma unroll
  for (int i = 0; i < 3; i++) {
    M[i][0] = fmaf(C[i][2], r[1], -(C[i][1] * r[2]));
    M[i][1] = fmaf(C[i][0], r[2], -(C[i][2] * r[0]));
    M[i][2] = fmaf(C[i][1], r[0], -(C[i][0] * r[1]));
  }
  float dv[6];
#pragma unroll
  for (int k = 0; k < 6; k++) dv[k] = -d2f * v[k];
#pragma unroll
  for (int i = 0; i < 3; i++) {
#pragma unroll
    for (int j = i; j < 3; j++) a[fsym(i, j)] = fmaf(e, fmaf(dv[i], v[j], C[i][j]), a[fsym(i, j)]);
#pragma unroll
    for (int k = 0; k < 3; k++) a[fsym(i, 3 + k)] = fmaf(e, fmaf(dv[i], v[3 + k], M[i][k]), a[fsym(i, 3 + k)]);
  }
#pragma unroll
  for (int k = 0; k < 3; k++) {
    const float rr0 = fmaf(r[1], M[2][k], -(r[2] * M[1][k]));
    const float rr1 = fmaf(r[2], M[0][k], -(r[0] * M[2][k]));
    const float rr2 = fmaf(r[0], M[1][k], -(r[1] * M[0][k]));
    if (k >= 0) a[fsym(3, 3 + k)] = fmaf(e, fmaf(dv[3], v[3 + k], rr0), a[fsym(3, 3 + k)]);
    if (k >= 1) a[fsym(4, 3 + k)] = fmaf(e, fmaf(dv[4], v[3 + k], rr1), a[fsym(4, 3 + k)]);
    if (k >= 2) a[fsym(5, 3 + k)] = fmaf(e, fmaf(dv[5], v[3 + k], rr2), a[fsym(5, 3 + k)]);
  }
#pragma unroll
  for (int i = 0; i < 3; i++) {
    const float er = e * r[i];
#pragma unroll
    for (int j = 0; j < 3; j++) a[FA_BASE + 3 * i + j] = fmaf(er, y[j], a[FA_BASE + 3 * i + j]);
  }
}
__device__ __forceinline__ void fast_acc_to_row(const float a[NACC_F], double acc[43]) {
#pragma unroll
  for (int k = 0; k < 7; k++) acc[k] = (double)a[k];
  const double tr = ((double)a[FA_BASE] + (double)a[FA_BASE + 4]) + (double)a[FA_BASE + 8];
#pragma unroll
  for (int i = 0; i < 6; i++) {
#pragma unroll
    for (int j = 0; j < 6; j++) {
      double h = (double)a[fsym(i, j)];
      if (i >= 3 && j >= 3) { h += (double)a[FA_BASE + 3 * (i - 3) + (j - 3)]; if (i == j) h -= tr; }
      acc[7 + i * 6 + j] = h;
    }
  }
}

__host__ __device__ constexpr int probe_off(int K, int q, int a) {
  const int o7[7][3] = {{0,0,0},{1,0,0},{-1,0,0},{0,1,0},{0,-1,0},{0,0,1},{0,0,-1}};
  const int o26[26][3] = {{-1,-1,-1}, {-1,0,-1}, {-1,1,-1}, {0,-1,-1}, {0,0,-1}, {0,1,-1}, {1,-1,-1}, {1,0,-1}, {1,1,-1}, {-1,-1,0}, {0,-1,0}, {1,-1,0}, {-1,0,0}, {1,1,1}, {1,0,1}, {1,-1,1}, {0,1,1}, {0,0,1}, {0,-1,1}, {-1,1,1}, {-1,0,1}, {-1,-1,1}, {1,1,0}, {0,1,0}, {-1,1,0}, {1,0,0}};
  return K == 1 ? 0 : (K == 7 ? o7[q][a] : (K == 26 ? o26[q][a] : (a == 0 ? q % 3 - 1 : (a == 1 ? (q / 3) % 3 - 1 : q / 9 - 1))));
}

#define Q_GROUP 7
#define ID_BITS 23
#define WAVES   (SWEEP_THREADS / 64)

#ifdef NDT_TIMELINE
__device__ unsigned long long g_tl[16];
#define TL_STAMP(k) do { __builtin_amdgcn_sched_barrier(0); const unsigned long long t_ = __builtin_readcyclecounter(); tl[k] += t_ - tl_last; tl_last = t_; __builtin_amdgcn_sched_barrier(0); } while (0)
#else
#define TL_STAMP(k) do {} while (0)
#endif
struct SweepCtl {
  int n_active;
  int next_item[8];
};
#define QUARTERS WAVES

#ifndef FAST_WPE7
#define FAST_WPE7 4
#endif
#ifndef FAST_WPE1
#define FAST_WPE1 3
#endif
#ifndef FAST_TP7
#define FAST_TP7 1
#endif
#ifndef FAST_TP1
#define FAST_TP1 2
#endif
#ifndef FAST_PIPE
#define FAST_PIPE 1
#endif
template <bool PCA, int K, int ORD = 0>
struct SweepTune {
  static constexpr bool FAST = (ORD == 2);
  static constexpr bool LEAN = false;
  static constexpr int  WPE  = FAST ? (K == 1 ? FAST_WPE1 : FAST_WPE7) : (LEAN ? 3 : SWEEP_WPE);
  static constexpr bool PIPE = FAST ? (FAST_PIPE != 0) : !LEAN;
  static constexpr int  TP   = FAST ? (K == 1 ? FAST_TP1 : FAST_TP7) : (LEAN ? 1 : (K == 1 ? 8 : (K <= 7 ? 2 : 1)));
};
static inline int sweep_wpe(bool pca, int K, bool fast = false) { (void)pca; return fast ? (K == 1 ? FAST_WPE1 : FAST_WPE7) : SWEEP_WPE; }

typedef __attribute__((address_space(1))) unsigned int gu32;
typedef __attribute__((address_space(1))) unsigned long long gu64;
#define RLX_AGENT __ATOMIC_RELAXED, __HIP_MEMORY_SCOPE_AGENT
__device__ __forceinline__ unsigned sweep_pose_words(const PairState* S) {
  static_assert(offsetof(PairState, T) == 0 && offsetof(PairState, Rj) == 48, "pose words");
  const int lane = threadIdx.x & 63;
  unsigned w = 0;
  if (lane < 21) w = __hip_atomic_load((const gu32*)reinterpret_cast<const unsigned*>(S) + lane, RLX_AGENT);
  return w;
}

template <bool PCA, int NROWS, bool ASYNC>
__device__ __forceinline__ void sweep_rows_d1p(const int b, const int rem0, const float* __restrict__ src, const size_t pitch, const float T[12], const float Rj[9], const int n,
                                               const GridDesc& g, const BitWord* __restrict__ words, const VoxelRec* __restrict__ recs,
                                               double* partials, const int rows_per_pair, const SweepConst& sc
#ifdef NDT_TIMELINE
                                               , unsigned long long* tl, unsigned long long& tl_last
#endif
                                               );
#ifndef FAST_D1_POINT
#define FAST_D1_POINT 0
#endif

template <bool PCA, int K, int IT, bool FINE, int ORD, bool ASYNC>
__device__ __forceinline__ void sweep_item(const int b, const int rem, const float* __restrict__ src, const size_t pitch, const PairState* st,
                                           const GridDesc* __restrict__ gd, const BitWord* __restrict__ words, const VoxelRec* __restrict__ recs,
                                           double* partials, const int rows_per_pair, const SweepConst& sc, const float* __restrict__ cent,
                                           const int* __restrict__ grid_of, const double* exp_tab,
                                           const unsigned pose_w, const int n_async, const int g_async
#ifdef NDT_TIMELINE
                                           , unsigned long long* tl, unsigned long long& tl_last
#endif
                                           ) {
  constexpr bool KD = (K == 27);
  constexpr bool FAST = (ORD == 2);
  static_assert(!FAST || K == 1 || K == 7, "tolerance arithmetic is instantiated for DIRECT1 / DIRECT7");
  typedef SweepTune<PCA, K, ORD> Tune;
  const int lane = threadIdx.x & 63, wv = threadIdx.x >> 6;
  const unsigned long long lt_mask = (1ull << lane) - 1ull;
  constexpr bool PCAQ = PCA && K > 1;
  constexpr int TP = Tune::TP < IT ? Tune::TP : IT;
  constexpr int Q_NEED = (IT / TP > 1 ? 64 : 0) + TP * (K < Q_GROUP ? K : Q_GROUP) * 64;
  constexpr int Q_CAP = FAST ? (Q_NEED <= 128 ? 128 : Q_NEED <= 256 ? 256 : Q_NEED <= 512 ? 512 : 1024) : ((K > 1 && K <= Q_GROUP) ? 1024 : 512);
  static_assert(Q_NEED <= Q_CAP, "hit queue");
  __shared__ unsigned q_ent[WAVES][Q_CAP];
  typedef typename std::conditional<K == 1, int, typename std::conditional<FAST, float, double>::type>::type QW;
  __shared__ QW q_w[PCAQ ? WAVES : 1][PCAQ ? Q_CAP : 1];
  constexpr int NBUF = (IT / TP > 1) ? 2 : 1;
  __shared__ float stage[WAVES][NBUF * 64 * TP][6];

  __shared__ double red[FINE ? WAVES : 1][FINE ? NACC : 1];
  const PairState& S = st[b];
  const int n = ASYNC ? n_async : S.n_src;
  const GridDesc& g = gd[ASYNC ? g_async : (grid_of ? grid_of[b] : b)];
  const float* X = src + (size_t)b * 3 * pitch;
  const BitWord* W = words + g.word_off;
  const VoxelRec* R = recs + g.rec_off;
  const bool grid_ok = (g.status == GRID_OK);
  float T[12], Rj[9];
#pragma unroll
  for (int a = 0; a < 12; a++) T[a] = ASYNC ? __uint_as_float(__builtin_amdgcn_readlane(pose_w, a)) : S.T[a];
#pragma unroll
  for (int a = 0; a < 9; a++) Rj[a] = ASYNC ? __uint_as_float(__builtin_amdgcn_readlane(pose_w, 12 + a)) : S.Rj[a];
  if constexpr (FAST && K == 1 && IT == 8 && !FINE && FAST_D1_POINT) {
    sweep_rows_d1p<PCA, 1, ASYNC>(b, rem, src, pitch, T, Rj, n, g, words, recs, partials, rows_per_pair, sc
#ifdef NDT_TIMELINE
                                  , tl, tl_last
#endif
                                  );
    return;
  }
  const float leaf = g.leaf;
  const int mb0 = g.min_b[0], mb1 = g.min_b[1], mb2 = g.min_b[2];
  const int xb0 = g.max_b[0], xb1 = g.max_b[1], xb2 = g.max_b[2];
  const int mul1 = g.mul1, mul2 = g.mul2, nwords = g.nwords;
  {
    typedef typename std::conditional<FAST, float, double>::type AccT;
    AccT acc[FAST ? NACC_F : 43];
#pragma unroll
    for (int a = 0; a < (FAST ? NACC_F : 43); a++) acc[a] = (AccT)0;
    unsigned nhits = 0;
    int qhead = 0, qcount = 0;
    int q_old = 0;
    const int wbase = rem * (IT * 64);

    struct BatchX { unsigned slot; double m0, m1, m2; float C[9]; int weight; double w; };
    struct BatchF { unsigned slot; float mh[3], ml[3], c[6]; int weight; float w; };
    typedef typename std::conditional<FAST, BatchF, BatchX>::type Batch;
    auto fetch = [&](int off, int m, Batch& B) {
      const int k = lane < m ? lane : m - 1;
      const unsigned ent = q_ent[wv][(qhead + off + k) & (Q_CAP - 1)];
      B.slot = ent >> ID_BITS;
      if constexpr (FAST) {
        const VoxelRecF& vr = reinterpret_cast<const VoxelRecF*>(R)[ent & ((1u << ID_BITS) - 1)];
#pragma unroll
        for (int a = 0; a < 3; a++) { B.mh[a] = vr.mh[a]; B.ml[a] = vr.ml[a]; }
#pragma unroll
        for (int a = 0; a < 6; a++) B.c[a] = vr.c[a];
        B.weight = vr.weight;
        B.w = 1.f;
        if (PCAQ) B.w = (float)q_w[wv][(qhead + off + k) & (Q_CAP - 1)];
        else if (PCA) B.w = (float)vr.weight;
      } else {
        const VoxelRec& vr = R[ent & ((1u << ID_BITS) - 1)];
        B.m0 = vr.mean[0]; B.m1 = vr.mean[1]; B.m2 = vr.mean[2];
#pragma unroll
        for (int a = 0; a < 9; a++) B.C[a] = vr.icov[a];
        B.weight = vr.weight;
        B.w = 1.0;
        if (PCAQ) B.w = (double)q_w[wv][(qhead + off + k) & (Q_CAP - 1)];
        else if (PCA) B.w = (double)vr.weight;
      }
    };
    auto eval_batch = [&](const Batch& B, int m, auto mid) {
      const float* sp = stage[wv][B.slot];
      const float xt0 = sp[0], xt1 = sp[1], xt2 = sp[2];
      float r[3] = {sp[3], sp[4], sp[5]};
      const bool live = lane < m && (PCAQ || KD || B.weight != VOX_DEAD);
      if constexpr (FAST) {
        float u[3] = {(xt0 - B.mh[0]) - B.ml[0], (xt1 - B.mh[1]) - B.ml[1], (xt2 - B.mh[2]) - B.ml[2]};
        eval_hit_fast<PCA, decltype(mid)>(u, r, B.c, sc.d1f, sc.d2f, sc.kq, B.w, live, acc, mid);
      } else {
        float u[3] = {(float)((double)xt0 - B.m0), (float)((double)xt1 - B.m1), (float)((double)xt2 - B.m2)};
        eval_hit<PCA, decltype(mid), KD, ORD>(u, r, B.C, sc.d1, sc.d2f, B.w, live, acc, exp_tab, mid);
      }
      nhits += PCAQ ? (unsigned)m : (unsigned)__popcll(__ballot(live));
      qhead = (qhead + m) & (Q_CAP - 1);
      qcount -= m;
      q_old = q_old > m ? q_old - m : 0;
    };
    auto drain = [&](int m) {
      Batch B;
      fetch(0, m, B);
      eval_batch(B, m, NoHook());
    };
    auto drain_full = [&]() {
      if (!Tune::PIPE) {
        while (qcount >= 64) drain(64);
        return;
      }
      if (qcount < 64) return;
      Batch A;
      fetch(0, 64, A);
#pragma unroll 1
      for (;;) {
        const bool more = qcount >= 128;
        Batch N;
        eval_batch(A, 64, [&]() { if (more) fetch(64, 64, N); });
        if (!more) break;
        A = N;
      }
    };
    if (wbase < n && grid_ok) {
      constexpr int NST = IT / TP;
      const unsigned e0 = (unsigned)(xb0 - mb0), e1 = (unsigned)(xb1 - mb1), e2 = (unsigned)(xb2 - mb2);
      const unsigned empty_cell = (unsigned)(nwords - 1) << 6;
      float nx[TP], ny[TP], nz[TP];
#pragma unroll
      for (int p = 0; p < TP; p++) {
        const int i = wbase + p * 64 + lane;
        nx[p] = ny[p] = nz[p] = 0.f;
        if (i < n) { nx[p] = X[i]; ny[p] = X[pitch + i]; nz[p] = X[2 * pitch + i]; }
      }
      TL_STAMP(1);
#pragma unroll 1
      for (int st = 0; st < NST; st++) {
        if (wbase + st * TP * 64 >= n) break;
        if (q_old > 0) { __builtin_amdgcn_wave_barrier(); drain(q_old); }
        q_old = qcount;
        int r0[TP], r1[TP], r2[TP], cc[TP];
        bool valid[TP];
        float kx[TP], ky[TP], kz[TP];
#pragma unroll
        for (int p = 0; p < TP; p++) {
          const int i = wbase + (st * TP + p) * 64 + lane;
          const float px = nx[p], py = ny[p], pz = nz[p];
          const int inext = i + TP * 64;
// ... 33 lines not shown
              const int o0 = probe_off(K, q, 0), o1 = probe_off(K, q, 1), o2 = probe_off(K, q, 2);
              const bool inside = valid[p] && (unsigned)(r0[p] + o0) <= e0 && (unsigned)(r1[p] + o1) <= e1 && (unsigned)(r2[p] + o2) <= e2;
              cellv[p][j] = inside ? (unsigned)(cc[p] + o0 + o1 * mul1 + o2 * mul2) : empty_cell;
              bwv[p][j] = *reinterpret_cast<const uint4*>(W + (cellv[p][j] >> 6));
            }
          }
          TL_STAMP(3);
          unsigned idv[TP][Q_GROUP];
          int wiv[TP][Q_GROUP];
#pragma unroll
          for (int p = 0; p < TP; p++) {
#pragma unroll
            for (int j = 0; j < Q_GROUP; j++) {
              if (q1 - 1 - j < 0) continue;
              const unsigned long long bits = ((unsigned long long)bwv[p][j].y << 32) | bwv[p][j].x;
              const unsigned long long tb = bits << (63u - (cellv[p][j] & 63u));
              idv[p][j] = bwv[p][j].z + (unsigned)__popcll(tb) - 1u;
              wiv[p][j] = ((long long)tb < 0) ? 1 : VOX_DEAD;
              if (PCAQ) { if ((long long)tb < 0) wiv[p][j] = R[idv[p][j]].weight; }
              if (KD && (long long)tb < 0) {
                const float* cp = cent + 3 * (size_t)(g.rec_off + idv[p][j]);
                const float dx = kx[p] - cp[0], dy = ky[p] - cp[1], dz = kz[p] - cp[2];
                if (!(((dx * dx + dy * dy) + dz * dz) < sc.kd_r2)) wiv[p][j] = VOX_DEAD;
              }
            }
          }
#pragma unroll
          for (int p = 0; p < TP; p++) {
            const int slot = ((st & 1) * TP + p) * 64 + lane;
#pragma unroll
            for (int j = 0; j < Q_GROUP; j++) {
              if (q1 - 1 - j < 0) continue;
              const bool hit = wiv[p][j] != VOX_DEAD;
              if (PCAQ && hit) suf[p] *= (double)wiv[p][j];
              const unsigned long long mask = __ballot(hit);
              if (hit) {
                const int pos = (qhead + qcount + (int)__popcll(mask & lt_mask)) & (Q_CAP - 1);
                q_ent[wv][pos] = ((unsigned)slot << ID_BITS) | idv[p][j];
                if (PCAQ) q_w[wv][pos] = (QW)suf[p];
              }
              qcount += (int)__popcll(mask);
            }
          }
          __builtin_amdgcn_wave_barrier();
          TL_STAMP(4);
          drain_full();
          TL_STAMP(5);
        }
      }
      __builtin_amdgcn_wave_barrier();
      if (qcount > 0) drain(qcount);
      TL_STAMP(5);
    }
    typedef unsigned int u2v __attribute__((ext_vector_type(2)));
    double accd[43];
    if constexpr (FAST) fast_acc_to_row(acc, accd);
    else {
#pragma unroll
      for (int i = 0; i < 43; i++) accd[i] = acc[i];
    }
    double P1[22], P2[11];
#pragma unroll
    for (int i = 0; i < 22; i++) {
      const double a = accd[i], b2 = (i + 22 < 43) ? accd[i + 22] : 0.0;
      const u2v lo = __builtin_amdgcn_permlane32_swap((unsigned)__double2loint(a), (unsigned)__double2loint(b2), false, false);
      const u2v hi = __builtin_amdgcn_permlane32_swap((unsigned)__double2hiint(a), (unsigned)__double2hiint(b2), false, false);
      P1[i] = __hiloint2double((int)hi.x, (int)lo.x) + __hiloint2double((int)hi.y, (int)lo.y);
    }
#pragma unroll
    for (int i = 0; i < 11; i++) {
      const double a = P1[i], b2 = P1[i + 11];
      const u2v lo = __builtin_amdgcn_permlane16_swap((unsigned)__double2loint(a), (unsigned)__double2loint(b2), false, false);
      const u2v hi = __builtin_amdgcn_permlane16_swap((unsigned)__double2hiint(a), (unsigned)__double2hiint(b2), false, false);
      double v = __hiloint2double((int)hi.x, (int)lo.x) + __hiloint2double((int)hi.y, (int)lo.y);
#pragma unroll
      for (int o = 8; o > 0; o >>= 1) v += __shfl_xor(v, o);
      P2[i] = v;
    }
    if ((lane & 15) == 0) {
      const int row = lane >> 4, base = 11 * (row & 1) + 22 * (row >> 1);
      double* P = FINE ? &red[FINE ? wv : 0][0] : partials + ((size_t)b * rows_per_pair + rem) * NACC;
      if (ASYNC && !FINE) {
        gu64* PG = (gu64*)reinterpret_cast<unsigned long long*>(P);
#pragma unroll
        for (int i = 0; i < 11; i++) if (base + i < 43) __hip_atomic_store(PG + base + i, (unsigned long long)__double_as_longlong(P2[i]), RLX_AGENT);
        if (lane == 0) __hip_atomic_store(PG + 43, (unsigned long long)__double_as_longlong((double)nhits), RLX_AGENT);
      } else {
#pragma unroll
        for (int i = 0; i < 11; i++) if (base + i < 43) P[base + i] = P2[i];
        if (lane == 0) P[43] = (double)nhits;
      }
    }
    if (FINE) {
      __syncthreads();
      if (wv == 0 && lane < NACC)
        partials[((size_t)b * (rows_per_pair >> 2) + (rem >> 2)) * NACC + lane] = ((red[0][lane] + red[FINE ? 1 : 0][lane]) + red[FINE ? 2 : 0][lane]) + red[FINE ? 3 : 0][lane];
      __syncthreads();
    }
    TL_STAMP(6);
#ifdef NDT_TIMELINE
    tl[7] += 1;
#endif
  }
}

template <bool PCA, int ORD, int NROWS>
__device__ __forceinline__ void sweep_rows_d1(const int b, const int rem0, const float* __restrict__ src, const size_t pitch,
                                              const GridDesc* __restrict__ gd, const BitWord* __restrict__ words, const VoxelRec* __restrict__ recs,
                                              double* partials, const int rows_per_pair, const SweepConst& sc, const double* exp_tab,
                                              const unsigned pose_w, const int n, const int g_idx
#ifdef NDT_TIMELINE
                                              , unsigned long long* tl, unsigned long long& tl_last
#endif
                                              ) {
  constexpr int TP = 2, IT = 8, NST = IT / TP, Q_CAP = 512;
  const int lane = threadIdx.x & 63, wv = threadIdx.x >> 6;
  const unsigned long long lt_mask = (1ull << lane) - 1ull;
  __shared__ unsigned q_ent[WAVES][Q_CAP];
  __shared__ float stage[WAVES][64 * IT][6];
  const GridDesc& g = gd[g_idx];
  const float* X = src + (size_t)b * 3 * pitch;
  const BitWord* W = words + g.word_off;
  const VoxelRec* R = recs + g.rec_off;
  const bool grid_ok = (g.status == GRID_OK);
  float T[12], Rj[9];
#pragma unroll
  for (int a = 0; a < 12; a++) T[a] = __uint_as_float(__builtin_amdgcn_readlane(pose_w, a));
#pragma unroll
  for (int a = 0; a < 9; a++) Rj[a] = __uint_as_float(__builtin_amdgcn_readlane(pose_w, 12 + a));
  const float leaf = g.leaf;
  const int mb0 = g.min_b[0], mb1 = g.min_b[1], mb2 = g.min_b[2];
  const unsigned e0 = (unsigned)(g.max_b[0] - mb0), e1 = (unsigned)(g.max_b[1] - mb1), e2 = (unsigned)(g.max_b[2] - mb2);
  const int mul1 = g.mul1, mul2 = g.mul2;
  const int base = rem0 * (IT * 64);
  constexpr int S_TOTAL = NROWS * NST;

  double acc[43];
#pragma unroll
  for (int a = 0; a < 43; a++) acc[a] = 0.0;
  unsigned nhits = 0;
  int qhead = 0, qcount = 0;

  struct Batch { unsigned slot; double m0, m1, m2; float C[9]; int weight; };
  auto fetch = [&](int off, int m, Batch& B) {
    const int k = lane < m ? lane : m - 1;
    const unsigned ent = q_ent[wv][(qhead + off + k) & (Q_CAP - 1)];
    B.slot = ent >> ID_BITS;
    const VoxelRec& vr = R[ent & ((1u << ID_BITS) - 1)];
    B.m0 = vr.mean[0]; B.m1 = vr.mean[1]; B.m2 = vr.mean[2];
#pragma unroll
    for (int a = 0; a < 9; a++) B.C[a] = vr.icov[a];
    B.weight = vr.weight;
  };
  auto eval_batch = [&](const Batch& B, int m, auto mid) {
    const float* sp = stage[wv][B.slot];
    const float xt0 = sp[0], xt1 = sp[1], xt2 = sp[2];
    float r[3] = {sp[3], sp[4], sp[5]};
    const bool live = lane < m && B.weight != VOX_DEAD;
    float u[3] = {(float)((double)xt0 - B.m0), (float)((double)xt1 - B.m1), (float)((double)xt2 - B.m2)};
    eval_hit<PCA, decltype(mid), false, ORD>(u, r, B.C, sc.d1, sc.d2f, PCA ? (double)B.weight : 1.0, live, acc, exp_tab, mid);
    nhits += (unsigned)__popcll(__ballot(live));
    qhead = (qhead + m) & (Q_CAP - 1);
    qcount -= m;
  };
  auto drain_full = [&]() {
    if (qcount < 64) return;
    Batch A;
    fetch(0, 64, A);
#pragma unroll 1
    for (;;) {
      const bool more = qcount >= 128;
      Batch N;
      eval_batch(A, 64, [&]() { if (more) fetch(64, 64, N); });
      if (!more) break;
      A = N;
    }
  };

  float nx[TP], ny[TP], nz[TP];
  uint4 bw[TP];
  unsigned cellv[TP];
  auto load_points = [&](const int s) {
#pragma unroll
    for (int p = 0; p < TP; p++) {
      const int i = base + (s * TP + p) * 64 + lane;
      nx[p] = ny[p] = nz[p] = 0.f;
      if (s < S_TOTAL && i < n) { nx[p] = X[i]; ny[p] = X[pitch + i]; nz[p] = X[2 * pitch + i]; }
    }
  };
  auto probe = [&](const int s) {
#pragma unroll
    for (int p = 0; p < TP; p++) {
      const int i = base + (s * TP + p) * 64 + lane;
      const float px = nx[p], py = ny[p], pz = nz[p];
      bool ok = grid_ok && i < n && finite3(px, py, pz);
      float xt[3], r[3];
#pragma unroll
      for (int a = 0; a < 3; a++) {
        xt[a] = ((T[a * 4 + 0] * px + T[a * 4 + 1] * py) + T[a * 4 + 2] * pz) + T[a * 4 + 3];
        r[a] = (Rj[a * 3 + 0] * px + Rj[a * 3 + 1] * py) + Rj[a * 3 + 2] * pz;
      }
      ok = ok && finite3(xt[0], xt[1], xt[2]);
      float* sp = stage[wv][(((s % NST) * TP) + p) * 64 + lane];
      sp[0] = xt[0]; sp[1] = xt[1]; sp[2] = xt[2]; sp[3] = r[0]; sp[4] = r[1]; sp[5] = r[2];
      const int c0 = (int)floorf(sc.leaf_pow2 ? xt[0] * sc.inv_leaf : xt[0] / leaf);
      const int c1 = (int)floorf(sc.leaf_pow2 ? xt[1] * sc.inv_leaf : xt[1] / leaf);
      const int c2 = (int)floorf(sc.leaf_pow2 ? xt[2] * sc.inv_leaf : xt[2] / leaf);
      const int r0 = c0 - mb0, r1 = c1 - mb1, r2 = c2 - mb2;
      const bool inside = ok && (unsigned)r0 <= e0 && (unsigned)r1 <= e1 && (unsigned)r2 <= e2;
      cellv[p] = inside ? (unsigned)(r0 + r1 * mul1 + r2 * mul2) : 0u;
      bw[p] = make_uint4(0u, 0u, 0u, 0u);
      if (inside) bw[p] = *reinterpret_cast<const uint4*>(W + (cellv[p] >> 6));
    }
  };
  auto push = [&](const int s) {
#pragma unroll
    for (int p = 0; p < TP; p++) {
      const unsigned long long bits = ((unsigned long long)bw[p].y << 32) | bw[p].x;
      const unsigned long long tb = bits << (63u - (cellv[p] & 63u));
      const unsigned id = bw[p].z + (unsigned)__popcll(tb) - 1u;
      const bool hit = (long long)tb < 0;
      const unsigned long long mask = __ballot(hit);
      if (hit) {
        const int pos = (qhead + qcount + (int)__popcll(mask & lt_mask)) & (Q_CAP - 1);
        q_ent[wv][pos] = ((unsigned)((((s % NST) * TP) + p) * 64 + lane) << ID_BITS) | id;
      }
      qcount += (int)__popcll(mask);
    }
    __builtin_amdgcn_wave_barrier();
  };

  load_points(0);
  TL_STAMP(1);
  probe(0);
  load_points(1);
  TL_STAMP(2);
#pragma unroll 1
  for (int s = 0; s < S_TOTAL; s++) {
    const bool row_end = (s % NST) == NST - 1;
    push(s);
    TL_STAMP(4);
    if (!row_end) { probe(s + 1); load_points(s + 2); }
    drain_full();
    TL_STAMP(5);
    if (!row_end) continue;
    __builtin_amdgcn_wave_barrier();
    if (qcount > 0) { Batch Bt; fetch(0, qcount, Bt); eval_batch(Bt, qcount, NoHook()); }
    TL_STAMP(5);
    if (s + 1 < S_TOTAL) { probe(s + 1); load_points(s + 2); }
    typedef unsigned int u2v __attribute__((ext_vector_type(2)));
    double P1[22], P2[11];
#pragma unroll
    for (int i = 0; i < 22; i++) {
      const double a = acc[i], b2 = (i + 22 < 43) ? acc[i + 22] : 0.0;
      const u2v lo = __builtin_amdgcn_permlane32_swap((unsigned)__double2loint(a), (unsigned)__double2loint(b2), false, false);
      const u2v hi = __builtin_amdgcn_permlane32_swap((unsigned)__double2hiint(a), (unsigned)__double2hiint(b2), false, false);
      P1[i] = __hiloint2double((int)hi.x, (int)lo.x) + __hiloint2double((int)hi.y, (int)lo.y);
    }
#pragma unroll
    for (int i = 0; i < 11; i++) {
      const double a = P1[i], b2 = P1[i + 11];
      const u2v lo = __builtin_amdgcn_permlane16_swap((unsigned)__double2loint(a), (unsigned)__double2loint(b2), false, false);
      const u2v hi = __builtin_amdgcn_permlane16_swap((unsigned)__double2hiint(a), (unsigned)__double2hiint(b2), false, false);
      double v = __hiloint2double((int)hi.x, (int)lo.x) + __hiloint2double((int)hi.y, (int)lo.y);
#pragma unroll
      for (int o = 8; o > 0; o >>= 1) v += __shfl_xor(v, o);
      P2[i] = v;
    }
    if ((lane & 15) == 0) {
      const int row = lane >> 4, rb = 11 * (row & 1) + 22 * (row >> 1);
      gu64* PG = (gu64*)reinterpret_cast<unsigned long long*>(partials + ((size_t)b * rows_per_pair + rem0 + s / NST) * NACC);
#pragma unroll
      for (int i = 0; i < 11; i++) if (rb + i < 43) __hip_atomic_store(PG + rb + i, (unsigned long long)__double_as_longlong(P2[i]), RLX_AGENT);
      if (lane == 0) __hip_atomic_store(PG + 43, (unsigned long long)__double_as_longlong((double)nhits), RLX_AGENT);
    }
#pragma unroll
    for (int a = 0; a < 43; a++) acc[a] = 0.0;
    nhits = 0;
    TL_STAMP(6);
#ifdef NDT_TIMELINE
    tl[7] += 1;
#endif
  }
}

template <bool PCA, int NROWS, bool ASYNC>
__device__ __forceinline__ void sweep_rows_d1p(const int b, const int rem0, const float* __restrict__ src, const size_t pitch, const float T[12], const float Rj[9], const int n,
                                               const GridDesc& g, const BitWord* __restrict__ words, const VoxelRec* __restrict__ recs,
                                               double* partials, const int rows_per_pair, const SweepConst& sc
#ifdef NDT_TIMELINE
                                               , unsigned long long* tl, unsigned long long& tl_last
#endif
                                               ) {
  constexpr int IT = 8, S_TOTAL = NROWS * IT;
  const int lane = threadIdx.x & 63;
  const float* X = src + (size_t)b * 3 * pitch;
  const BitWord* W = words + g.word_off;
  const VoxelRecF* R = reinterpret_cast<const VoxelRecF*>(recs) + g.rec_off;
  const bool grid_ok = (g.status == GRID_OK);
  const float leaf = g.leaf;
  const int mb0 = g.min_b[0], mb1 = g.min_b[1], mb2 = g.min_b[2];
  const unsigned e0 = (unsigned)(g.max_b[0] - mb0), e1 = (unsigned)(g.max_b[1] - mb1), e2 = (unsigned)(g.max_b[2] - mb2);
  const int mul1 = g.mul1, mul2 = g.mul2;
  const int base = rem0 * (IT * 64);

  float acc[NACC_F];
#pragma unroll
  for (int a = 0; a < NACC_F; a++) acc[a] = 0.f;
  unsigned nhits = 0;
  float px = 0.f, py = 0.f, pz = 0.f;
  float axt[3] = {0.f, 0.f, 0.f}, ar[3] = {0.f, 0.f, 0.f}; unsigned acell = 0u; bool ain = false; uint4 abw = make_uint4(0u, 0u, 0u, 0u);
  float bxt[3] = {0.f, 0.f, 0.f}, br[3] = {0.f, 0.f, 0.f}; bool bhit = false;
  float4 q0 = make_float4(0.f, 0.f, 0.f, 0.f), q1 = q0, q2 = q0; int bweight = 0;
  auto load_points = [&](const int s) {
    const int i = base + s * 64 + lane;
    px = py = pz = 0.f;
    if (s < S_TOTAL && i < n) { px = X[i]; py = X[pitch + i]; pz = X[2 * pitch + i]; }
  };
  auto probe = [&](const int s) {
    const int i = base + s * 64 + lane;
    bool ok = grid_ok && s < S_TOTAL && i < n && finite3(px, py, pz);
#pragma unroll
    for (int a = 0; a < 3; a++) {
      axt[a] = ((T[a * 4 + 0] * px + T[a * 4 + 1] * py) + T[a * 4 + 2] * pz) + T[a * 4 + 3];
      ar[a] = fmaf(Rj[a * 3 + 2], pz, fmaf(Rj[a * 3 + 1], py, Rj[a * 3 + 0] * px));
    }
    ok = ok && finite3(axt[0], axt[1], axt[2]);
// ... 179 lines not shown
```

### lv_slam_amd/csrc/ndt_types.hpp

```cpp
#pragma once
#include <hip/hip_runtime.h>
#include <climits>
#include <cstddef>
#include <cstring>
#include "mi355_ndt.h"

#ifdef NDT_SECOND_TU
#define NDT_KERNEL static __global__
#else
#define NDT_KERNEL __global__
#endif

#define CHUNK_PTS      2048
#define SWEEP_THREADS  256
#ifndef SWEEP_WPE
#define SWEEP_WPE       2
#endif
#define NACC           44
#define MAX_CELLS      (1 << 25)

enum { GRID_OK = 0, GRID_EMPTY = 1, GRID_OVERFLOW = 2, GRID_CAP = 3 };
enum { PH_SWEEP0 = 0, PH_STEP = 1, PH_DONE = 2, PH_HESS = 3 };

struct GridDesc {
  int   min_b[3], max_b[3], div_b[3];
  int   mul1, mul2;
  float leaf, inv_leaf;
  int   ncells, nwords;
  int   status;
  int   n_voxels;
  unsigned word_off;
  unsigned rec_off;
};

struct BitWord {
  unsigned long long bits;
  unsigned prefix;
  unsigned pad;
};

struct VoxelRec {
  double mean[3];
  float  icov[9];
  int    weight;
};
#define VOX_DEAD INT_MIN

struct alignas(16) VoxelRecF {
  float mh[3], ml[3];
  float c[6];
  float pad_[3];
  int   weight;
};
static_assert(sizeof(VoxelRecF) == sizeof(VoxelRec) && offsetof(VoxelRecF, weight) == offsetof(VoxelRec, weight), "the two record forms share slot size and weight word");

struct PairState {
  float  T[12];
  float  Rj[9];
  double p[6];
  double dir[6];
  double a_t;
  double score, g[6], H[36];
  double trans_probability;
  long long hits;
  float  final_cm[16];
  int    it, phase, converged, sweeps, n_src, grid_status;
  double xt[6], phi0, dphi0;
  int    mt_loops, pad_;
  float  inc_cm[16], prev_inc_cm[16];
  double reb_pn[6];
  float  reb_inc[16];
  long long reb_tag;
};

struct SweepConst {
  double d1;
  float  d2f;
  int    K;
  int    pca;
  int    table;
  float  kd_r2;
  int    leaf_pow2;
  float  inv_leaf;
  int    dyn_shift;
  volatile int* host_flags;
  int    seq_no;
  int    rebase_block;
  float  d1f, kq;
};

__constant__ int c_off[3][26][3] = {
  {{0,0,0}},
  {{0,0,0},{1,0,0},{-1,0,0},{0,1,0},{0,-1,0},{0,0,1},{0,0,-1}},
  {{-1,-1,-1}, {-1,0,-1}, {-1,1,-1}, {0,-1,-1}, {0,0,-1}, {0,1,-1}, {1,-1,-1}, {1,0,-1}, {1,1,-1}, {-1,-1,0}, {0,-1,0}, {1,-1,0}, {-1,0,0}, {1,1,1}, {1,0,1}, {1,-1,1}, {0,1,1}, {0,0,1}, {0,-1,1}, {-1,1,1}, {-1,0,1}, {-1,-1,1}, {1,1,0}, {0,1,0}, {-1,1,0}, {1,0,0}}
};

__device__ __forceinline__ int f2ord(float f) { int i = __float_as_int(f); return i >= 0 ? i : i ^ 0x7FFFFFFF; }
__device__ __forceinline__ float ord2f(int i) { return __int_as_float(i >= 0 ? i : i ^ 0x7FFFFFFF); }

__device__ __forceinline__ bool grid_too_big(float e0, float e1, float e2) {
  const float e[3] = {e0, e1, e2};
  double prod = 1.0;
  for (int a = 0; a < 3; a++) {
    if (!(e[a] < 2147483648.0f)) return true;
    prod *= (double)((long long)e[a] + 1);
  }
  return prod > 2147483647.0;
}
__device__ __forceinline__ bool finite3(float x, float y, float z) { return isfinite(x) && isfinite(y) && isfinite(z); }

__device__ __forceinline__ bool xcd_map(int nx, int n_targets, int& bx, int& b) {
  const int L = blockIdx.x, xcd = L & 7, s = L >> 3;
  b = xcd + 8 * (s / nx);
  bx = s % nx;
  return b < n_targets;
}
static inline unsigned xcd_grid(int nx, int n_targets) { return 8u * (unsigned)((n_targets + 7) / 8) * (unsigned)nx; }


template <int NT>
__device__ __forceinline__ unsigned block_exscan(unsigned v, unsigned* total, unsigned* sm) {
  const int lane = threadIdx.x & 63, w = threadIdx.x >> 6;
  unsigned inc = v;
#pragma unroll
  for (int o = 1; o < 64; o <<= 1) { const unsigned t = __shfl_up(inc, o); if (lane >= o) inc += t; }
  if (lane == 63) sm[w] = inc;
// ... 16 lines not shown
```

### lv_slam_amd/csrc/ndt_update.hpp

```cpp
#pragma once
#include "ndt_types.hpp"
#include "ndt_math.hpp"
#include "ndt_sweep.hpp"

__device__ void finalize_pair(PairState& S, mi355ndt_result* res, int converged) {
  S.converged = converged;
  S.phase = PH_DONE;
  S.trans_probability = S.score / (double)S.n_src;
  mi355ndt_result o;
  for (int a = 0; a < 16; a++) o.final_colmajor[a] = S.final_cm[a];
  o.trans_probability = S.trans_probability;
  o.score = S.score;
  o.iterations = S.it;
  o.converged = converged;
  o.sweeps = S.sweeps;
  o.status = (S.grid_status == GRID_OK || S.grid_status == GRID_EMPTY) ? MI355NDT_OK : MI355NDT_ERR_GRID;
  o.hits_last = S.hits;
  *res = o;
}

__device__ inline void set_increment_se3(PairState& S, const ndtm::SE3& e) {
  double R[9];
  ndtm::q_to_matrix(e.q, R);
  for (int r = 0; r < 3; r++) {
    for (int c = 0; c < 3; c++) S.inc_cm[c * 4 + r] = (float)R[r * 3 + c];
    S.inc_cm[12 + r] = (float)e.t[r];
    S.inc_cm[r * 4 + 3] = 0.f;
  }
  S.inc_cm[15] = 1.f;
}
__device__ inline void set_increment(PairState& S, const double dp[6]) { set_increment_se3(S, ndtm::se3_exp(dp)); }

__device__ __forceinline__ double shfl_d(double v, int src) { return __shfl(v, src); }
__device__ __forceinline__ ndtm::SE3 shfl_se3(const ndtm::SE3& e, int src) {
  ndtm::SE3 r;
  r.q.w = shfl_d(e.q.w, src); r.q.x = shfl_d(e.q.x, src); r.q.y = shfl_d(e.q.y, src); r.q.z = shfl_d(e.q.z, src);
  r.t[0] = shfl_d(e.t[0], src); r.t[1] = shfl_d(e.t[1], src); r.t[2] = shfl_d(e.t[2], src);
  return r;
}

__device__ inline void init_pair_state(PairState& S, const float G[16] , int n_src, int grid_status) {
  double R[9], t[3];
  for (int r = 0; r < 3; r++) {
    for (int c = 0; c < 3; c++) { S.T[r * 4 + c] = G[c * 4 + r]; R[r * 3 + c] = (double)G[c * 4 + r]; }
    S.T[r * 4 + 3] = G[12 + r];
    t[r] = (double)G[12 + r];
  }
  for (int a = 0; a < 16; a++) S.final_cm[a] = G[a];
  ndtm::se3_log(ndtm::se3_from_Rt(R, t), S.p);
  float Tdummy[12];
  ndtm::pose_to_f32(S.p, Tdummy, S.Rj);
  S.it = 0; S.phase = PH_SWEEP0; S.converged = 0; S.sweeps = 1; S.a_t = 0; S.hits = 0; S.score = 0; S.mt_loops = 0;
  for (int a = 0; a < 16; a++) S.inc_cm[a] = S.prev_inc_cm[a] = (a % 5 == 0) ? 1.f : 0.f;
  S.n_src = n_src;
  S.grid_status = grid_status;
  S.reb_tag = -1;
}

NDT_KERNEL void k_init_state(PairState* st, const float* __restrict__ guess_cm, const int* __restrict__ src_cnt,
                             const GridDesc* __restrict__ gd, int n_pairs, int* active_list, SweepCtl* ctl) {
  int b = blockIdx.x * blockDim.x + threadIdx.x;
  if (b >= n_pairs) return;
  active_list[b] = b;
  if (b == 0) ctl->n_active = n_pairs;
  init_pair_state(st[b], guess_cm + (size_t)b * 16, src_cnt[b], gd[b].status);
}

NDT_KERNEL void k_set_pose(PairState* st, int b, const float* __restrict__ T_cm, const float* __restrict__ Rj, const int* __restrict__ src_cnt,
                           const GridDesc* __restrict__ gd, int* active_list, SweepCtl* ctl) {
  PairState& S = st[b];
  active_list[0] = b; ctl->n_active = 1;
  for (int r = 0; r < 3; r++) for (int c = 0; c < 4; c++) S.T[r * 4 + c] = T_cm[c * 4 + r];
  for (int a = 0; a < 9; a++) S.Rj[a] = Rj[a];
  S.phase = PH_SWEEP0; S.n_src = src_cnt[b]; S.grid_status = gd[b].status; S.it = 0; S.sweeps = 1;
}
NDT_KERNEL void k_set_pose_p(PairState* st, int b, const double* __restrict__ p, const int* __restrict__ src_cnt, const GridDesc* __restrict__ gd,
                             int* active_list, SweepCtl* ctl, int for_hessian) {
  PairState& S = st[b];
  active_list[0] = b; ctl->n_active = 1;
  double pp[6];
  for (int a = 0; a < 6; a++) { pp[a] = p[a]; S.xt[a] = p[a]; }
  ndtm::pose_to_f32(pp, S.T, S.Rj);
  S.phase = for_hessian ? PH_HESS : PH_SWEEP0; S.n_src = src_cnt[b]; S.grid_status = gd[b].status; S.it = 0; S.sweeps = 1;
}

__device__ inline double mt_cmin(double a, double b) { return b < a ? b : a; }
__device__ inline double mt_cmax(double a, double b) { return a < b ? b : a; }

__device__ inline bool mt_update_interval(double I[6], double a_t, double f_t, double g_t) {
  if (f_t > I[1]) { I[3] = a_t; I[4] = f_t; I[5] = g_t; return false; }
  if (g_t * (I[0] - a_t) > 0) { I[0] = a_t; I[1] = f_t; I[2] = g_t; return false; }
  if (g_t * (I[0] - a_t) < 0) { I[3] = I[0]; I[4] = I[1]; I[5] = I[2]; I[0] = a_t; I[1] = f_t; I[2] = g_t; return false; }
  return true;
}

__device__ inline double mt_trial_value(const double I[6], double a_t, double f_t, double g_t) {
  const double a_l = I[0], f_l = I[1], g_l = I[2], a_u = I[3], f_u = I[4], g_u = I[5];
  if (f_t > f_l) {
    const double z = 3 * (f_t - f_l) / (a_t - a_l) - g_t - g_l;
    const double w = sqrt(z * z - g_t * g_l);
    const double a_c = a_l + (a_t - a_l) * (w - g_l - z) / (g_t - g_l + 2 * w);
    const double a_q = a_l - 0.5 * (a_l - a_t) * g_l / (g_l - (f_l - f_t) / (a_l - a_t));
    return fabs(a_c - a_l) < fabs(a_q - a_l) ? a_c : 0.5 * (a_q + a_c);
  }
  if (g_t * g_l < 0) {
    const double z = 3 * (f_t - f_l) / (a_t - a_l) - g_t - g_l;
    const double w = sqrt(z * z - g_t * g_l);
    const double a_c = a_l + (a_t - a_l) * (w - g_l - z) / (g_t - g_l + 2 * w);
    const double a_s = a_l - (a_l - a_t) / (g_l - g_t) * g_l;
    return fabs(a_c - a_t) >= fabs(a_s - a_t) ? a_c : a_s;
  }
  if (fabs(g_t) <= fabs(g_l)) {
    const double z = 3 * (f_t - f_l) / (a_t - a_l) - g_t - g_l;
    const double w = sqrt(z * z - g_t * g_l);
    const double a_c = a_l + (a_t - a_l) * (w - g_l - z) / (g_t - g_l + 2 * w);
    const double a_s = a_l - (a_l - a_t) / (g_l - g_t) * g_l;
    const double a_n = fabs(a_c - a_t) < fabs(a_s - a_t) ? a_c : a_s;
    return a_t > a_l ? mt_cmin(a_t + 0.66 * (a_u - a_t), a_n) : mt_cmax(a_t + 0.66 * (a_u - a_t), a_n);
  }
  const double z = 3 * (f_t - f_u) / (a_t - a_u) - g_t - g_u;
  const double w = sqrt(z * z - g_t * g_u);
  return a_u + (a_t - a_u) * (w - g_u - z) / (g_t - g_u + 2 * w);
}

__device__ inline int mt_loop(PairState& S, double step_max, double step_min) {
  const double mu = 1.e-4, nu = 0.9;
  const double phi_0 = S.phi0, d_phi_0 = S.dphi0;
  double I[6] = {0, phi_0 - phi_0 - mu * d_phi_0 * 0.0, d_phi_0 - mu * d_phi_0, 0, phi_0 - phi_0 - mu * d_phi_0 * 0.0, d_phi_0 - mu * d_phi_0};
  bool interval_converged = (step_max - step_min) > 0, open_interval = true;
  double a_t = S.a_t;
  const double score_c = S.score;
  double g_c[6];
  for (int a = 0; a < 6; a++) g_c[a] = S.g[a];
  double score = score_c, gd = 0;
  for (int a = 0; a < 6; a++) gd += g_c[a] * S.dir[a];
  double phi_t = -score, d_phi_t = -gd;
// ... 87 lines not shown

enum { NEWTON_DONE = 0, NEWTON_SWEEP = 1, NEWTON_HESSIAN = 2 };

__device__ __forceinline__ void newton_solve(const PairState& S, double d[6]) {
  double neg[6];
  for (int a = 0; a < 6; a++) neg[a] = -S.g[a];
  bool fin = true;
  for (int a = 0; a < 36; a++) fin = fin && isfinite(S.H[a]);
  for (int a = 0; a < 6; a++) fin = fin && isfinite(S.g[a]);
  if (!fin || !ndtm::lu_solve6(S.H, neg, d)) ndtm::svd_solve6(S.H, neg, d);
}
#define SOL_WORDS 8
__device__ __forceinline__ void newton_solve_side(const PairState& S, volatile double* sol) {
  const int lane = threadIdx.x & 63;
  if (lane > 6) return;
  double rhs[6], x[6];
  for (int a = 0; a < 6; a++) rhs[a] = lane < 6 ? (a == lane ? 1.0 : 0.0) : -S.g[a];
  bool fin = true;
  for (int a = 0; a < 36; a++) fin = fin && isfinite(S.H[a]);
  for (int a = 0; a < 6; a++) fin = fin && isfinite(S.g[a]);
  double pmin, pmax;
  bool ok = fin && ndtm::lu_solve6_rhs(S.H, rhs, x, pmin, pmax);
  const double c2 = (ok && lane < 6) ? ndtm::norm2_6(x) : 0.0;
  const double r2 = lane < 6 ? ndtm::norm2_6(S.H + 6 * lane) : 0.0;
  double hF2 = 0, invF2 = 0;
  for (int k = 0; k < 6; k++) { invF2 += __shfl(c2, k); hF2 += __shfl(r2, k); }
  if (lane != 6) return;
  ok = ok && ndtm::lu_accept(hF2, invF2);
  if (!ok) ndtm::svd_solve6(S.H, rhs, x);
  for (int a = 0; a < 6; a++) sol[a] = x[a];
  __threadfence_block();
  sol[6] = 1.0;
}

__device__ __forceinline__ void newton_rebase(const double p[6], const double dir[6], const double a_t, double pn[6], float inc_cm[16]) {
  const int lane = threadIdx.x & 63;
  double in[6];
  for (int a = 0; a < 6; a++) in[a] = (lane & 1) ? p[a] : dir[a] * a_t;
  const ndtm::SE3 e = ndtm::se3_exp(in);
  const ndtm::SE3 e_dp = shfl_se3(e, 0), e_p = shfl_se3(e, 1);
  double R[9];
  ndtm::q_to_matrix(e_dp.q, R);
  for (int r = 0; r < 3; r++) {
    for (int c = 0; c < 3; c++) inc_cm[c * 4 + r] = (float)R[r * 3 + c];
    inc_cm[12 + r] = (float)e_dp.t[r];
    inc_cm[r * 4 + 3] = 0.f;
  }
  inc_cm[15] = 1.f;
  ndtm::se3_log(ndtm::se3_mul(e_dp, e_p), pn);
}

__device__ __forceinline__ int newton_update(PairState& S, mi355ndt_result* res, double step_max, double eps, int max_iterations, int mt,
                                             volatile double* sol = nullptr ,
                                             const bool rebased = false ) {
  const int lane = threadIdx.x & 63;
  ndtm::SE3 e_dp, e_p;
  const bool pre = (mt == 0) && (S.phase == PH_STEP) && !rebased;
  if (pre) {
    double in[6];
    for (int a = 0; a < 6; a++) in[a] = (lane & 1) ? S.p[a] : S.dir[a] * S.a_t;
    const ndtm::SE3 e = ndtm::se3_exp(in);
    e_dp = shfl_se3(e, 0);
    e_p = shfl_se3(e, 1);
  }
  if (lane != 0) return NEWTON_DONE;

  const double step_min = eps / 2;
  if (mt == 1 && S.phase == PH_STEP) {
    const int its = mt_loop(S, step_max, step_min);
    S.mt_loops += its;
    S.sweeps += its;
    if (its) {
      bool fin = S.a_t == S.a_t;
      if (!fin) {
        for (int a = 0; a < 6; a++) S.xt[a] = S.p[a] + S.dir[a] * S.a_t;
        ndtm::pose_to_f32(S.xt, S.T, S.Rj);
        for (int r = 0; r < 3; r++) {
          for (int c = 0; c < 4; c++) S.final_cm[c * 4 + r] = S.T[r * 4 + c];
          S.final_cm[r * 4 + 3] = 0.f;
        }
        S.final_cm[15] = 1.f;
        S.score = 0; S.hits = 0;
        for (int a = 0; a < 6; a++) S.g[a] = 0;
        for (int a = 0; a < 36; a++) S.H[a] = 0;
      } else {
        S.phase = PH_HESS;
        return NEWTON_HESSIAN;
      }
    }
  }
  if (S.phase == PH_HESS) S.phase = PH_STEP;
  if (S.phase == PH_STEP) {
    double pn[6];
    if (rebased) {
      for (int a = 0; a < 16; a++) S.inc_cm[a] = S.reb_inc[a];
      for (int a = 0; a < 6; a++) pn[a] = S.reb_pn[a];
    } else if (pre) {
      set_increment_se3(S, e_dp);
      ndtm::se3_log(ndtm::se3_mul(e_dp, e_p), pn);
    } else {
      double dp[6];
      for (int a = 0; a < 6; a++) dp[a] = S.dir[a] * S.a_t;
      const ndtm::SE3 ed = ndtm::se3_exp(dp);
      set_increment_se3(S, ed);
      ndtm::se3_log(ndtm::se3_mul(ed, ndtm::se3_exp(S.p)), pn);
    }
    for (int a = 0; a < 6; a++) S.p[a] = pn[a];
    const bool conv = (S.it > max_iterations) || (S.it && (fabs(S.a_t) < eps));
    S.it++;
    if (conv) { finalize_pair(S, res, 1); return NEWTON_DONE; }
  }
  for (int guard = 0; guard < 4; guard++) {
    for (int a = 0; a < 16; a++) S.prev_inc_cm[a] = S.inc_cm[a];
    double d[6];
    if (sol) {
      while (sol[6] == 0.0) __builtin_amdgcn_s_sleep(1);
      __threadfence_block();
      for (int a = 0; a < 6; a++) d[a] = sol[a];
    } else {
      newton_solve(S, d);
    }
    double nrm = 0;
    for (int a = 0; a < 6; a++) nrm += d[a] * d[a];
    nrm = sqrt(nrm);
    if (nrm == 0 || nrm != nrm) { finalize_pair(S, res, nrm == nrm); return NEWTON_DONE; }
    for (int a = 0; a < 6; a++) d[a] /= nrm;
    double dphi0 = 0;
    for (int a = 0; a < 6; a++) dphi0 += S.g[a] * d[a];
    dphi0 = -dphi0;
    if (dphi0 >= 0 && dphi0 == 0) {
      double z[6] = {0, 0, 0, 0, 0, 0}, pn[6];
      set_increment(S, z);
      ndtm::se3_log(ndtm::se3_mul(ndtm::se3_exp(z), ndtm::se3_exp(S.p)), pn);
      for (int a = 0; a < 6; a++) S.p[a] = pn[a];
      const bool conv = (S.it > max_iterations) || (S.it && (0.0 < eps));
      S.it++;
      if (conv) { finalize_pair(S, res, 1); return NEWTON_DONE; }
      continue;
    }
    if (dphi0 >= 0) { for (int a = 0; a < 6; a++) d[a] = -d[a]; }
    double a_t = nrm;
    a_t = a_t < step_max ? a_t : step_max;
    a_t = a_t > step_min ? a_t : step_min;
    double xt[6];
    for (int a = 0; a < 6; a++) { S.dir[a] = d[a]; xt[a] = S.p[a] + d[a] * a_t; S.xt[a] = xt[a]; }
    S.a_t = a_t;
    S.phi0 = -S.score;
    S.dphi0 = dphi0 >= 0 ? -dphi0 : dphi0;
    ndtm::pose_to_f32(xt, S.T, S.Rj);
    for (int r = 0; r < 3; r++) {
      for (int c = 0; c < 4; c++) S.final_cm[c * 4 + r] = S.T[r * 4 + c];
      S.final_cm[r * 4 + 3] = 0.f;
    }
    S.final_cm[15] = 1.f;
    S.phase = PH_STEP;
    S.sweeps++;
    return NEWTON_SWEEP;
  }
  finalize_pair(S, res, 1);
  return NEWTON_DONE;
}

NDT_KERNEL void __launch_bounds__(UPD_THREADS, 2)
k_update(PairState* st, const double* __restrict__ partials, int rows_per_pair, int pts_per_chunk, int chunk_rows, mi355ndt_result* results,
         int* active_counter, int* active_list, SweepCtl* ctl, unsigned long long* hits_total,
         double step_max, double eps, int max_iterations, int reduce_only, int mt) {
  __shared__ double sm[UPD_WAVES][NACC];
  __shared__ double sol[SOL_WORDS];
  __shared__ PairState Ssh;
  const int b = blockIdx.x;
  static_assert(sizeof(PairState) % 8 == 0, "PairState travels as 8-byte words");
  constexpr int NW = (int)(sizeof(PairState) / 8);
  unsigned long long* sg = reinterpret_cast<unsigned long long*>(&st[b]);
  unsigned long long* sl = reinterpret_cast<unsigned long long*>(&Ssh);
  for (int i = threadIdx.x; i < NW; i += UPD_THREADS) sl[i] = sg[i];
  if (threadIdx.x == 0) sol[6] = 0.0;
  __syncthreads();
  PairState& S = Ssh;
  if (S.phase == PH_DONE) return;
  if (mt == 2 && S.phase != PH_HESS) return;
  const int lane = threadIdx.x & 63;
  const int nchunks = (S.n_src + pts_per_chunk - 1) / pts_per_chunk;
  const bool take = (mt != 2 || (lane >= 7 && lane < 43));
  const double v = reduce_pair_rows(partials + (size_t)b * rows_per_pair * NACC, nchunks, take, sm, chunk_rows != 0);
  if (threadIdx.x < NACC && take) {
    if (lane == 0) S.score = v;
    else if (lane < 7) S.g[lane - 1] = v;
    else if (lane < 43) S.H[lane - 7] = v;
    else { S.hits = (long long)v; if (hits_total) atomicAdd(hits_total, (unsigned long long)v); }
  }
  __syncthreads();
  if (threadIdx.x >= 128) return;
  if (threadIdx.x >= 64) { if (mt == 0 && !reduce_only) newton_solve_side(S, sol); return; }
  if (!reduce_only) {
    const bool rebased = mt == 0 && S.phase == PH_STEP && S.reb_tag == (long long)S.sweeps;
    const int rc = newton_update(S, &results[b], step_max, eps, max_iterations, mt, mt == 0 ? sol : nullptr, rebased);
    if (lane == 0 && rc == NEWTON_SWEEP) {
      atomicAdd(active_counter, 1);
      active_list[atomicAdd(&ctl->n_active, 1)] = b;
// ... 55 lines not shown
```

### lv_slam_amd/ndt.py

```python
from __future__ import annotations

import ctypes as C
import os
import numpy as np

_HERE = os.path.dirname(os.path.abspath(__file__))
LIB_PATH = os.environ.get("MI355NDT_LIB") or os.path.join(_HERE, "libmi355ndt.so")

KDTREE, DIRECT26, DIRECT7, DIRECT1 = 0, 1, 2, 3
VARIANT_OMP, VARIANT_PCA = 0, 1

OK = 0
ERR = {-1: "bad handle", -2: "bad argument", -3: "HIP error", -4: "target grid unusable", -5: "no HIP device",
       -6: "unsupported configuration", -7: "target/source not set"}


class NDTError(RuntimeError):
    def __init__(self, code, where, detail=""):
        self.code = code
        super().__init__(f"{where}: {ERR.get(code, code)}" + (f" ({detail})" if detail else ""))


class Params(C.Structure):
    _fields_ = [("resolution", C.c_float), ("step_size", C.c_double), ("outlier_ratio", C.c_double),
                ("trans_epsilon", C.c_double), ("max_iterations", C.c_int), ("neighbor_mode", C.c_int),
                ("variant", C.c_int), ("min_points_per_voxel", C.c_int), ("min_covar_eigvalue_mult", C.c_double)]


class Result(C.Structure):
    _fields_ = [("final_colmajor", C.c_float * 16), ("trans_probability", C.c_double), ("score", C.c_double),
                ("iterations", C.c_int), ("converged", C.c_int), ("sweeps", C.c_int), ("status", C.c_int),
                ("hits_last", C.c_longlong)]


class Voxel(C.Structure):
    _fields_ = [("idx", C.c_int32), ("n", C.c_int32), ("mean", C.c_double * 3), ("icov", C.c_float * 9),
                ("weight", C.c_int32)]


class Profile(C.Structure):
    _fields_ = [("sweep_ms", C.c_double), ("sweep_launches", C.c_longlong), ("sweep_alg_bytes", C.c_double),
                ("sweep_hits", C.c_longlong), ("sweep_points", C.c_longlong), ("build_ms", C.c_double),
                ("build_launches", C.c_longlong), ("build_alg_bytes", C.c_double), ("update_ms", C.c_double),
                ("update_launches", C.c_longlong), ("async_fallbacks", C.c_longlong), ("stream_launches", C.c_longlong),
                ("stream_carried", C.c_longlong), ("stream_redone", C.c_longlong), ("cloud_uploads", C.c_longlong), ("cloud_upload_bytes", C.c_longlong),
                ("cloud_transfers", C.c_longlong), ("cloud_promotions", C.c_longlong),
                ("stream_reserved_slots", C.c_longlong), ("stream_launch_slots", C.c_longlong)]


class SeqParams(C.Structure):
    _fields_ = [("keyframe_delta_trans", C.c_double), ("keyframe_delta_angle", C.c_double), ("keyframe_delta_time", C.c_double)]


class SeqFrame(C.Structure):
    _fields_ = [("odom_colmajor", C.c_double * 16), ("tf_s2k_colmajor", C.c_float * 16), ("trans_probability", C.c_double),
                ("dx", C.c_double), ("da", C.c_double), ("dt", C.c_double), ("key_id", C.c_int), ("new_keyframe", C.c_int),
                ("iterations", C.c_int), ("converged", C.c_int), ("aligns", C.c_int), ("pad", C.c_int)]


class SeqStats(C.Structure):
    _fields_ = [("upload_ms", C.c_double), ("build_ms", C.c_double), ("track_ms", C.c_double), ("aligns", C.c_longlong),
                ("update_launches", C.c_longlong)]


SYMBOLS = [
    "mi355ndt_version", "mi355ndt_device_count", "mi355ndt_host_numa_node", "mi355ndt_default_params", "mi355ndt_create", "mi355ndt_destroy",
    "mi355ndt_set_params", "mi355ndt_get_params", "mi355ndt_set_stream", "mi355ndt_last_error",
    "mi355ndt_set_target", "mi355ndt_set_source", "mi355ndt_promote_source_to_target", "mi355ndt_align", "mi355ndt_get_aligned", "mi355ndt_get_incremental",
    "mi355ndt_get_fitness_score", "mi355ndt_fitness_score_T", "mi355ndt_prefilter", "mi355ndt_use_prefiltered", "mi355ndt_derivatives", "mi355ndt_compute_hessian", "mi355ndt_derivatives_T", "mi355ndt_get_grid", "mi355ndt_get_voxels",
    "mi355ndt_batch_reserve", "mi355ndt_batch_set_target", "mi355ndt_batch_set_source", "mi355ndt_batch_set_clouds", "mi355ndt_batch_bind_device",
    "mi355ndt_batch_build_targets", "mi355ndt_batch_align", "mi355ndt_batch_size", "mi355ndt_batch_pose_records", "mi355ndt_batch_fitness_scores",
    "mi355ndt_profile_enable", "mi355ndt_profile_reset", "mi355ndt_profile_get", "mi355ndt_synchronize",
    "mi355ndt_set_latency_mode", "mi355ndt_sequence_run",
    "mi355ndt_calculate_score", "mi355ndt_convert_transform", "mi355ndt_set_option", "mi355ndt_get_option",
    "mi355ndt_stream_begin", "mi355ndt_stream_submit", "mi355ndt_stream_submit_host", "mi355ndt_stream_collect", "mi355ndt_stream_end", "mi355ndt_stream_pose_records", "mi355ndt_pack_pose_records",
]
OPT_ASYNC_ALIGN = 2
OPT_DEBUG_ASYNC_ABORT = 3
OPT_DEBUG_ASYNC_RINGS = 6
OPT_STREAM_RESERVE = 5
OPT_STREAM_THRESHOLD = 4
WARN_TOLERANCE_ARITH = 1
OPT_ARITH = 7
OPT_F32_SUM_ORDER = 1

_LIB = None


def load_library(path: str = LIB_PATH):
    global _LIB
    if _LIB is not None:
        return _LIB
    if not os.path.exists(path):
        raise ImportError(f"{path} not found: build it with `python -c 'import __graft_entry__ as g; g.build()'` "
                          "(hipcc --offload-arch=gfx950).  There is no CPU fallback.")
    L = C.CDLL(path)
    vp, i, sz = C.c_void_p, C.c_int, C.c_size_t
    L.mi355ndt_version.restype = C.c_char_p
    L.mi355ndt_last_error.restype = C.c_char_p
    L.mi355ndt_last_error.argtypes = [vp]
    L.mi355ndt_default_params.argtypes = [C.POINTER(Params)]
    L.mi355ndt_host_numa_node.argtypes = [i]
    L.mi355ndt_create.argtypes = [C.POINTER(Params), i, C.POINTER(vp)]
    L.mi355ndt_destroy.argtypes = [vp]
    L.mi355ndt_set_params.argtypes = [vp, C.POINTER(Params)]
    L.mi355ndt_get_params.argtypes = [vp, C.POINTER(Params)]
    L.mi355ndt_set_stream.argtypes = [vp, vp]
    L.mi355ndt_set_target.argtypes = [vp, vp, sz, sz]
    L.mi355ndt_set_source.argtypes = [vp, vp, sz, sz]
    L.mi355ndt_promote_source_to_target.argtypes = [vp]
    L.mi355ndt_align.argtypes = [vp, vp, C.POINTER(Result)]
    L.mi355ndt_get_aligned.argtypes = [vp, vp, sz]
    L.mi355ndt_get_incremental.argtypes = [vp, i, vp, vp]
    L.mi355ndt_get_fitness_score.argtypes = [vp, C.c_double, vp, vp]
    L.mi355ndt_fitness_score_T.argtypes = [vp, vp, C.c_double, vp, vp]
    L.mi355ndt_prefilter.argtypes = [vp, vp, sz, sz, i, C.c_double, C.c_double, C.c_float, vp, sz, sz, C.POINTER(sz)]
    L.mi355ndt_use_prefiltered.argtypes = [vp, i]
    L.mi355ndt_derivatives.argtypes = [vp, vp, vp, vp, vp, vp]
    L.mi355ndt_derivatives_T.argtypes = [vp, vp, vp, vp, vp, vp, vp]
    L.mi355ndt_compute_hessian.argtypes = [vp, vp, vp]
    L.mi355ndt_get_grid.argtypes = [vp, i, vp, vp, vp, vp]
    L.mi355ndt_get_voxels.argtypes = [vp, i, vp, sz]
    L.mi355ndt_batch_reserve.argtypes = [vp, i, sz, sz]
    L.mi355ndt_batch_set_target.argtypes = [vp, i, vp, sz, sz]
    L.mi355ndt_batch_set_source.argtypes = [vp, i, vp, sz, sz]
    L.mi355ndt_batch_set_clouds.argtypes = [vp, i, i, vp, vp, vp, vp, sz, i]
    L.mi355ndt_batch_bind_device.argtypes = [vp, i, vp, vp, sz, vp, vp, sz]
    L.mi355ndt_batch_build_targets.argtypes = [vp]
    L.mi355ndt_batch_align.argtypes = [vp, vp, vp]
    L.mi355ndt_batch_size.argtypes = [vp]
    L.mi355ndt_batch_pose_records.argtypes = [vp, i, i, vp, sz]
    L.mi355ndt_batch_fitness_scores.argtypes = [vp, vp, C.c_double, vp, vp]
    L.mi355ndt_profile_enable.argtypes = [vp, i]
    L.mi355ndt_profile_reset.argtypes = [vp]
    L.mi355ndt_profile_get.argtypes = [vp, C.POINTER(Profile)]
    L.mi355ndt_synchronize.argtypes = [vp]
    L.mi355ndt_set_latency_mode.argtypes = [vp, i]
# ... 466 lines not shown
```

Measured before the change: 60350.

## Evaluate only the score on the final NDT sweep, skipping gradient and Hessian

When the Newton step that was just chosen will end the pair (iteration limit reached or step below epsilon), the pair state is marked as a last sweep. Sweep kernels then take a score-only template path that evaluates just the Gaussian score and hit count, reduce them with a wave shuffle tree, and skip the 43-term gradient/Hessian accumulation, its stores, and the Newton solve. This removes derivative work on one sweep per pair, at the cost of more template instantiations, a new PairState field, and the requirement that the last-sweep prediction always matches real convergence.

Result: faster. 64990 (median of 6 runs) (+7.7%).

```diff
diff --git a/include/mi355_ndt.h b/include/mi355_ndt.h
--- a/include/mi355_ndt.h
+++ b/include/mi355_ndt.h
@@ -74,6 +74,7 @@
   long long cloud_promotions;
   long long stream_reserved_slots;
   long long stream_launch_slots;
+  long long score_only_sweeps;
 } mi355ndt_profile;
 
 typedef struct mi355ndt_handle mi355ndt_handle;
@@ -116,7 +117,8 @@
   MI355NDT_OPT_STREAM_THRESHOLD = 4,
   MI355NDT_OPT_STREAM_RESERVE = 5,
   MI355NDT_OPT_DEBUG_ASYNC_RINGS = 6,
-  MI355NDT_OPT_ARITH = 7
+  MI355NDT_OPT_ARITH = 7,
+  MI355NDT_OPT_SCORE_ONLY_LAST_SWEEP = 8
 };
 int mi355ndt_set_option(mi355ndt_handle* h, int option, int value);
 int mi355ndt_get_option(const mi355ndt_handle* h, int option, int* value);
diff --git a/lv_slam_amd/csrc/mi355_ndt.hip b/lv_slam_amd/csrc/mi355_ndt.hip
--- a/lv_slam_amd/csrc/mi355_ndt.hip
+++ b/lv_slam_amd/csrc/mi355_ndt.hip
@@ -92,6 +92,7 @@
   int items_per_pair = 0;
   bool async_force = false;
   bool async_align = true;
+  int score_only_last = 1;
   int* d_ring = nullptr; size_t ring_cap_total = 0; unsigned* d_arrived = nullptr; size_t arrived_cap = 0; AsyncCtl* d_actl = nullptr;
   AsyncCtl* h_pin_actl = nullptr;
   AsyncTab* d_atab = nullptr;
@@ -359,6 +360,7 @@
   if (const char* e = std::getenv("MI355NDT_FINE_TILES")) { const int v = std::atoi(e); if (v == 1 || v == 2) h->fine_tiles = v; }
   if (const char* e = std::getenv("MI355NDT_ARITH")) h->arith = std::atoi(e) == 1 ? 1 : 0;
   if (const char* e = std::getenv("MI355NDT_ASYNC")) { h->async_align = std::atoi(e) != 0; h->async_force = std::atoi(e) == 2; }
+  if (const char* e = std::getenv("MI355NDT_SCORE_ONLY_LAST_SWEEP")) h->score_only_last = std::atoi(e) != 0;
   if (const char* e = std::getenv("MI355NDT_SWEEP_DYN_SHIFT")) { const int v = std::atoi(e); if (v >= 0 && v <= 30) h->dyn_shift = v; }
   if (hipSetDevice(device) != hipSuccess || hipStreamCreateWithFlags(&h->stream, hipStreamNonBlocking) != hipSuccess) {
     delete h;
@@ -368,7 +370,8 @@
       hipHostMalloc((void**)&h->h_pin_active, 128 * sizeof(int)) != hipSuccess ||
       hipMalloc((void**)&h->d_active, 128 * sizeof(int)) != hipSuccess ||
       hipMalloc((void**)&h->d_ctl, 2 * sizeof(SweepCtl)) != hipSuccess ||
-      hipMalloc((void**)&h->d_hits, sizeof(unsigned long long)) != hipSuccess ||
+      hipMalloc((void**)&h->d_hits, 2 * sizeof(unsigned long long)) != hipSuccess ||
+      hipMemsetAsync(h->d_hits, 0, 2 * sizeof(unsigned long long), h->stream) != hipSuccess ||
       hipMalloc((void**)&h->d_hook, 64 * sizeof(double)) != hipSuccess ||
       hipEventCreateWithFlags(&h->ev_compute, hipEventDisableTiming) != hipSuccess ||
       hipEventCreateWithFlags(&h->ev_burst[0], hipEventDisableTiming) != hipSuccess ||
@@ -771,7 +774,7 @@
     e->P = mi355ndt_profile{};
   }
   h->P = mi355ndt_profile{};
-  (void)hipMemsetAsync(h->d_hits, 0, sizeof(unsigned long long), h->stream);
+  (void)hipMemsetAsync(h->d_hits, 0, 2 * sizeof(unsigned long long), h->stream);
   (void)hipStreamSynchronize(h->stream);
   return MI355NDT_OK;
 }
@@ -792,12 +795,13 @@
       h->P.cloud_uploads += e->P.cloud_uploads; e->P.cloud_uploads = 0; h->P.cloud_upload_bytes += e->P.cloud_upload_bytes; e->P.cloud_upload_bytes = 0;
       h->P.cloud_transfers += e->P.cloud_transfers; e->P.cloud_transfers = 0; }
   }
-  unsigned long long hh = 0;
-  HIPCHK(h, hipMemcpy(&hh, h->d_hits, sizeof hh, hipMemcpyDeviceToHost));
+  unsigned long long hh[2] = {0, 0};
+  HIPCHK(h, hipMemcpy(hh, h->d_hits, sizeof hh, hipMemcpyDeviceToHost));
   *out = h->P;
   if (h->stream_on) { out->stream_reserved_slots = h->s_reserve_wg; out->stream_launch_slots = h->s_launch_slots; }
-  out->sweep_hits += (long long)hh;
-  out->sweep_alg_bytes += 64.0 * (double)hh;
+  out->sweep_hits += (long long)hh[0];
+  out->sweep_alg_bytes += 64.0 * (double)hh[0];
+  out->score_only_sweeps = (long long)hh[1];
   return MI355NDT_OK;
 }
 
@@ -1179,7 +1183,7 @@
   SweepConst sc;
   make_sweep_const(e, sc);
   c.src = e->d_src; c.pitch = e->src_pitch; c.st = e->d_state; c.gd = e->d_grid; c.words = e->d_words; c.recs = sweep_recs(e, sc); c.cent = e->d_cent;
-  c.partials = e->d_partials; c.src_cnt = e->d_src_cnt; c.arrived = e->d_arrived; c.results = e->d_results; c.n_done = nullptr; c.must_finish = 1; c.pose = nullptr; c.pose_base = 0; c.pose_stride = 0; c.pad_ = 0;
+  c.partials = e->d_partials; c.src_cnt = e->d_src_cnt; c.arrived = e->d_arrived; c.results = e->d_results; c.n_done = nullptr; c.must_finish = 1; c.pose = nullptr; c.pose_base = 0; c.pose_stride = 0; c.score_only = e->score_only_last;
 }
 extern "C" {
 static int align_async(mi355ndt_handle* h, const SweepConst& sc, int B, mi355ndt_result* out) {
@@ -1829,7 +1833,8 @@
 
 int mi355ndt_set_option(mi355ndt_handle* h, int option, int value) {
   if (!h) return MI355NDT_ERR_BAD_HANDLE;
-  if (h->stream_on && (option == MI355NDT_OPT_F32_SUM_ORDER || option == MI355NDT_OPT_ARITH || option == MI355NDT_OPT_ASYNC_ALIGN)) NOT_IN_STREAM(h);
+  if (h->stream_on && (option == MI355NDT_OPT_F32_SUM_ORDER || option == MI355NDT_OPT_ARITH || option == MI355NDT_OPT_ASYNC_ALIGN ||
+                       option == MI355NDT_OPT_SCORE_ONLY_LAST_SWEEP)) NOT_IN_STREAM(h);
   if (option == MI355NDT_OPT_F32_SUM_ORDER) {
     if (value != 0 && value != 1) return MI355NDT_ERR_BAD_ARG;
     h->f32_sum_order = value;
@@ -1846,6 +1851,11 @@
     h->async_force = value == 2;
     return MI355NDT_OK;
   }
+  if (option == MI355NDT_OPT_SCORE_ONLY_LAST_SWEEP) {
+    if (value != 0 && value != 1) return MI355NDT_ERR_BAD_ARG;
+    h->score_only_last = value;
+    return MI355NDT_OK;
+  }
   if (option == MI355NDT_OPT_DEBUG_ASYNC_ABORT) {
     h->debug_abort_pos = value < 0 ? 0xFFFFFFFFu : (unsigned)value;
     return MI355NDT_OK;
@@ -1873,6 +1883,7 @@
   if (option == MI355NDT_OPT_F32_SUM_ORDER) { *value = h->f32_sum_order; return MI355NDT_OK; }
   if (option == MI355NDT_OPT_ARITH) { *value = h->arith; return MI355NDT_OK; }
   if (option == MI355NDT_OPT_ASYNC_ALIGN) { *value = h->async_force ? 2 : (h->async_align ? 1 : 0); return MI355NDT_OK; }
+  if (option == MI355NDT_OPT_SCORE_ONLY_LAST_SWEEP) { *value = h->score_only_last; return MI355NDT_OK; }
   if (option == MI355NDT_OPT_DEBUG_ASYNC_ABORT) { *value = h->debug_abort_pos == 0xFFFFFFFFu ? -1 : (int)h->debug_abort_pos; return MI355NDT_OK; }
   if (option == MI355NDT_OPT_DEBUG_ASYNC_RINGS) { *value = (int)h->debug_ring_mask; return MI355NDT_OK; }
   if (option == MI355NDT_OPT_STREAM_THRESHOLD) { *value = h->s_thresh_opt; return MI355NDT_OK; }
@@ -2115,7 +2126,7 @@
     }
     rc = mi355ndt_set_stream(e, h->s_reserve_wg > 0 ? h->s_build_stream : h->stream);
     if (rc) return fail(rc);
-    e->f32_sum_order = h->f32_sum_order; e->arith = h->arith; e->async_align = h->async_align; e->dyn_shift = h->dyn_shift;
+    e->f32_sum_order = h->f32_sum_order; e->arith = h->arith; e->async_align = h->async_align; e->dyn_shift = h->dyn_shift; e->score_only_last = h->score_only_last;
     e->async_build = true;
     e->ev_pool_target = 128;
     rc = ensure_pair_arrays(e, max_pairs);
diff --git a/lv_slam_amd/csrc/ndt_async.hpp b/lv_slam_amd/csrc/ndt_async.hpp
--- a/lv_slam_amd/csrc/ndt_async.hpp
+++ b/lv_slam_amd/csrc/ndt_async.hpp
@@ -16,7 +16,8 @@
   double* partials; const int* src_cnt; unsigned* arrived; mi355ndt_result* results;
   unsigned* n_done;
   int must_finish;
-  int pose_base; PoseRecord* pose; int pose_stride, pad_;
+  int pose_base; PoseRecord* pose; int pose_stride;
+  int score_only;
 };
 struct AsyncTab { AsyncCtx c[ASYNC_MAX_CTX]; };
 #define NDT_GP(T) __attribute__((address_space(1))) T*
@@ -26,7 +27,7 @@
   NDT_GP(double) partials; NDT_GP(const int) src_cnt; NDT_GP(unsigned) arrived; NDT_GP(mi355ndt_result) results;
   NDT_GP(unsigned) n_done;
   int must_finish;
-  int pose_base; NDT_GP(PoseRecord) pose; int pose_stride, pad_;
+  int pose_base; NDT_GP(PoseRecord) pose; int pose_stride, score_only;
 };
 static_assert(sizeof(AsyncCtxG) == sizeof(AsyncCtx) && offsetof(AsyncCtxG, pose) == offsetof(AsyncCtx, pose) && offsetof(AsyncCtxG, n_done) == offsetof(AsyncCtx, n_done),
               "AsyncCtxG mirrors AsyncCtx");
@@ -36,7 +37,7 @@
   c.src = (const float*)g.src; c.pitch = g.pitch; c.st = (PairState*)g.st; c.gd = (const GridDesc*)g.gd; c.words = (const BitWord*)g.words;
   c.recs = (const VoxelRec*)g.recs; c.cent = (const float*)g.cent; c.partials = (double*)g.partials; c.src_cnt = (const int*)g.src_cnt;
   c.arrived = (unsigned*)g.arrived; c.results = (mi355ndt_result*)g.results; c.n_done = (unsigned*)g.n_done; c.must_finish = g.must_finish;
-  c.pose_base = g.pose_base; c.pose = (PoseRecord*)g.pose; c.pose_stride = g.pose_stride; c.pad_ = 0;
+  c.pose_base = g.pose_base; c.pose = (PoseRecord*)g.pose; c.pose_stride = g.pose_stride; c.score_only = g.score_only;
   return c;
 }
 struct CtxStat { unsigned done, total_words, max_cells, plan_exceeded; };
@@ -168,13 +169,17 @@
   }
   asm volatile("s_waitcnt lgkmcnt(0)" ::: "memory");
   __builtin_amdgcn_wave_barrier();
-  if (lane < NACC) {
+  const bool last = __builtin_amdgcn_readfirstlane(Ssh.last_sweep) != 0;
+  if (lane < NACC && (!last || lane == 0 || lane == NACC - 1)) {
     double v = 0.0;
     v += aw0; v += aw1; v += aw2; v += aw3;
     if (lane == 0) Ssh.score = v;
     else if (lane < 7) Ssh.g[lane - 1] = v;
     else if (lane < 43) Ssh.H[lane - 7] = v;
-    else { Ssh.hits = (long long)v; if (hits_total) atomicAdd(hits_total, (unsigned long long)v); }
+    else {
+      Ssh.hits = (long long)v;
+      if (hits_total) { atomicAdd(hits_total, (unsigned long long)v); if (last) atomicAdd(hits_total + 1, 1ull); }
+    }
   }
   asm volatile("s_waitcnt lgkmcnt(0)" ::: "memory");
   __builtin_amdgcn_wave_barrier();
@@ -185,7 +190,11 @@
   bool reb_ok = want_reb && Ssh.reb_tag == (long long)Ssh.sweeps;
   unsigned long long rbw = 0;
   if (reb_ok && lane < 14) rbw = __hip_atomic_load(sg + RB0 + lane, RLX_AGENT);
-  newton_solve_side(Ssh, sol);
+  if (!last) newton_solve_side(Ssh, sol);
+  else if (lane == 0) {
+    for (int a = 0; a < 6; a++) sol[a] = 0.0;
+    sol[6] = 1.0;
+  }
   asm volatile("s_waitcnt lgkmcnt(0)" ::: "memory");
   __builtin_amdgcn_wave_barrier();
   TL_STAMP(13);
@@ -203,7 +212,7 @@
   asm volatile("s_waitcnt lgkmcnt(0)" ::: "memory");
   __builtin_amdgcn_wave_barrier();
   const bool rebased = reb_ok;
-  int rc = newton_update(Ssh, &results[b], step_max, eps, max_iterations, 0, sol, rebased);
+  int rc = newton_update(Ssh, &results[b], step_max, eps, max_iterations, 0, sol, rebased, C.score_only != 0);
   rc = __builtin_amdgcn_readfirstlane(rc);
   asm volatile("s_waitcnt lgkmcnt(0)" ::: "memory");
   __builtin_amdgcn_wave_barrier();
@@ -371,32 +380,37 @@
 #ifndef ASYNC_D1_PIPE
 #define ASYNC_D1_PIPE 1
 #endif
-    if constexpr (K == 1 && ASYNC_D1_PIPE && ORD != 2) {
-      sweep_rows_d1<PCA, ORD, CLAIM_D1>(b, rem, C.src, C.pitch, C.gd, C.words, C.recs, C.partials, I, sc, exp_tab, pose_w, n_b, b
-#ifdef NDT_TIMELINE
-                                     , tl, tl_last
-#endif
-                                     );
-    } else if constexpr (K == 1 && ORD == 2 && FAST_D1_POINT) {
-      float T[12], Rj[9];
-#pragma unroll
-      for (int a_ = 0; a_ < 12; a_++) T[a_] = __uint_as_float(__builtin_amdgcn_readlane(pose_w, a_));
-#pragma unroll
-      for (int a_ = 0; a_ < 9; a_++) Rj[a_] = __uint_as_float(__builtin_amdgcn_readlane(pose_w, 12 + a_));
-      sweep_rows_d1p<PCA, CLAIM_D1, true>(b, rem, C.src, C.pitch, T, Rj, n_b, C.gd[b], C.words, C.recs, C.partials, I, sc
-#ifdef NDT_TIMELINE
-                                          , tl, tl_last
-#endif
-                                          );
-    } else {
+    const bool last = __builtin_amdgcn_readlane(pose_w, POSE_W_LAST) != 0;
+    auto items = [&](auto so_c) {
+      constexpr bool SO = decltype(so_c)::value;
+      if constexpr (K == 1 && ASYNC_D1_PIPE && ORD != 2) {
+        sweep_rows_d1<PCA, ORD, CLAIM_D1, SO>(b, rem, C.src, C.pitch, C.gd, C.words, C.recs, C.partials, I, sc, exp_tab, pose_w, n_b, b
+#ifdef NDT_TIMELINE
+                                       , tl, tl_last
+#endif
+                                       );
+      } else if constexpr (K == 1 && ORD == 2 && FAST_D1_POINT) {
+        float T[12], Rj[9];
+#pragma unroll
+        for (int a_ = 0; a_ < 12; a_++) T[a_] = __uint_as_float(__builtin_amdgcn_readlane(pose_w, a_));
+#pragma unroll
+        for (int a_ = 0; a_ < 9; a_++) Rj[a_] = __uint_as_float(__builtin_amdgcn_readlane(pose_w, 12 + a_));
+        sweep_rows_d1p<PCA, CLAIM_D1, true>(b, rem, C.src, C.pitch, T, Rj, n_b, C.gd[b], C.words, C.recs, C.partials, I, sc
+#ifdef NDT_TIMELINE
+                                            , tl, tl_last
+#endif
+                                            );
+      } else {
 #pragma unroll 1
-      for (int k = 0; k < CLAIM; k++)
-        sweep_item<PCA, K, 8, false, ORD, true>(b, rem + k, C.src, C.pitch, C.st, C.gd, C.words, C.recs, C.partials, I, sc, C.cent, nullptr, exp_tab, pose_w, n_b, b
-#ifdef NDT_TIMELINE
-                                                , tl, tl_last
-#endif
-                                                );
-    }
+        for (int k = 0; k < CLAIM; k++)
+          sweep_item<PCA, K, 8, false, ORD, true, SO>(b, rem + k, C.src, C.pitch, C.st, C.gd, C.words, C.recs, C.partials, I, sc, C.cent, nullptr, exp_tab, pose_w, n_b, b
+#ifdef NDT_TIMELINE
+                                                  , tl, tl_last
+#endif
+                                                  );
+      }
+    };
+    if (last) items(std::true_type()); else items(std::false_type());
     unsigned npos = held_pos;
     if (lane == 0 && !held) npos = __hip_atomic_fetch_add(pos_p, 1u, RLX_AGENT);
     held = false;
diff --git a/lv_slam_amd/csrc/ndt_sweep.hpp b/lv_slam_amd/csrc/ndt_sweep.hpp
--- a/lv_slam_amd/csrc/ndt_sweep.hpp
+++ b/lv_slam_amd/csrc/ndt_sweep.hpp
@@ -76,6 +76,21 @@
     }
   }
 #undef NDT_ACC
+}
+
+template <bool PCA, int ORD = 0>
+__device__ __forceinline__ void eval_score(const float u[3], const float C[9], const double d1, const float d2f, const double w, const bool ok_in,
+                                           double& acc0, const double* __restrict__ exp_tab) {
+  float y[3];
+#pragma unroll
+  for (int j = 0; j < 3; j++) y[j] = sum3<ORD>(u[0] * C[j], u[1] * C[3 + j], u[2] * C[6 + j]);
+  const float qf = sum3<ORD>(u[0] * y[0], u[1] * y[1], u[2] * y[2]);
+  const float e0 = ndtm::exp_f32arg((-d2f * qf) * 0.5f, exp_tab);
+  float s_inc = (float)(-d1 * (double)e0);
+  const float e1 = d2f * e0;
+  const bool ok = ok_in && !(e1 > 1.f || e1 < 0.f || e1 != e1);
+  s_inc = ok ? s_inc : 0.f;
+  if (PCA) acc0 = fma(w, (double)s_inc, acc0); else acc0 += (double)s_inc;
 }
 
 #define NACC_F 37
@@ -138,6 +153,29 @@
     for (int j = 0; j < 3; j++) a[FA_BASE + 3 * i + j] = fmaf(er, y[j], a[FA_BASE + 3 * i + j]);
   }
 }
+template <bool PCA>
+__device__ __forceinline__ void eval_score_fast(const float u[3], const float c[6], const float d1f, const float d2f, const float kq,
+                                                const float w, const bool ok_in, float& a0) {
+  const float c00 = c[0], c01 = c[1], c02 = c[2], c11 = c[3], c12 = c[4], c22 = c[5];
+  float y[3];
+  y[0] = fmaf(c02, u[2], fmaf(c01, u[1], c00 * u[0]));
+  y[1] = fmaf(c12, u[2], fmaf(c11, u[1], c01 * u[0]));
+  y[2] = fmaf(c22, u[2], fmaf(c12, u[1], c02 * u[0]));
+  const float q = fmaf(u[2], y[2], fmaf(u[1], y[1], u[0] * y[0]));
+  const float e0 = __builtin_amdgcn_exp2f(kq * q);
+  const float e1 = d2f * e0;
+  const bool ok = ok_in && !(e1 > 1.f || e1 < 0.f || e1 != e1);
+  float s = -d1f * e0;
+  if (PCA) s *= w;
+  s = ok ? s : 0.f;
+  a0 += s;
+}
+__device__ __forceinline__ double score_tree(double v) {
+#pragma unroll
+  for (int o = 32; o > 0; o >>= 1) v += __shfl_xor(v, o);
+  return v;
+}
+
 __device__ __forceinline__ void fast_acc_to_row(const float a[NACC_F], double acc[43]) {
 #pragma unroll
   for (int k = 0; k < 7; k++) acc[k] = (double)a[k];
@@ -203,11 +241,12 @@
 typedef __attribute__((address_space(1))) unsigned int gu32;
 typedef __attribute__((address_space(1))) unsigned long long gu64;
 #define RLX_AGENT __ATOMIC_RELAXED, __HIP_MEMORY_SCOPE_AGENT
+#define POSE_W_LAST 21
 __device__ __forceinline__ unsigned sweep_pose_words(const PairState* S) {
-  static_assert(offsetof(PairState, T) == 0 && offsetof(PairState, Rj) == 48, "pose words");
+  static_assert(offsetof(PairState, T) == 0 && offsetof(PairState, Rj) == 48 && offsetof(PairState, last_sweep) == 4 * POSE_W_LAST, "pose words");
   const int lane = threadIdx.x & 63;
   unsigned w = 0;
-  if (lane < 21) w = __hip_atomic_load((const gu32*)reinterpret_cast<const unsigned*>(S) + lane, RLX_AGENT);
+  if (lane <= POSE_W_LAST) w = __hip_atomic_load((const gu32*)reinterpret_cast<const unsigned*>(S) + lane, RLX_AGENT);
   return w;
 }
 
@@ -219,11 +258,13 @@
                                                , unsigned long long* tl, unsigned long long& tl_last
 #endif
                                                );
+template <typename T, int SLOT>
+__device__ __forceinline__ T& item_lds() { __shared__ T v; return v; }
 #ifndef FAST_D1_POINT
 #define FAST_D1_POINT 0
 #endif
 
-template <bool PCA, int K, int IT, bool FINE, int ORD, bool ASYNC>
+template <bool PCA, int K, int IT, bool FINE, int ORD, bool ASYNC, bool SO = false>
 __device__ __forceinline__ void sweep_item(const int b, const int rem, const float* __restrict__ src, const size_t pitch, const PairState* st,
                                            const GridDesc* __restrict__ gd, const BitWord* __restrict__ words, const VoxelRec* __restrict__ recs,
                                            double* partials, const int rows_per_pair, const SweepConst& sc, const float* __restrict__ cent,
@@ -235,6 +276,7 @@
                                            ) {
   constexpr bool KD = (K == 27);
   constexpr bool FAST = (ORD == 2);
+  static_assert(!SO || (ASYNC && !FINE), "score-only items belong to the one-launch align");
   static_assert(!FAST || K == 1 || K == 7, "tolerance arithmetic is instantiated for DIRECT1 / DIRECT7");
   typedef SweepTune<PCA, K, ORD> Tune;
   const int lane = threadIdx.x & 63, wv = threadIdx.x >> 6;
@@ -244,13 +286,13 @@
   constexpr int Q_NEED = (IT / TP > 1 ? 64 : 0) + TP * (K < Q_GROUP ? K : Q_GROUP) * 64;
   constexpr int Q_CAP = FAST ? (Q_NEED <= 128 ? 128 : Q_NEED <= 256 ? 256 : Q_NEED <= 512 ? 512 : 1024) : ((K > 1 && K <= Q_GROUP) ? 1024 : 512);
   static_assert(Q_NEED <= Q_CAP, "hit queue");
-  __shared__ unsigned q_ent[WAVES][Q_CAP];
+  auto& q_ent = item_lds<unsigned[WAVES][Q_CAP], 0>();
   typedef typename std::conditional<K == 1, int, typename std::conditional<FAST, float, double>::type>::type QW;
-  __shared__ QW q_w[PCAQ ? WAVES : 1][PCAQ ? Q_CAP : 1];
+  auto& q_w = item_lds<QW[PCAQ ? WAVES : 1][PCAQ ? Q_CAP : 1], 1>();
   constexpr int NBUF = (IT / TP > 1) ? 2 : 1;
-  __shared__ float stage[WAVES][NBUF * 64 * TP][6];
-
-  __shared__ double red[FINE ? WAVES : 1][FINE ? NACC : 1];
+  auto& stage = item_lds<float[WAVES][NBUF * 64 * TP][6], 2>();
+
+  auto& red = item_lds<double[FINE ? WAVES : 1][FINE ? NACC : 1], 3>();
   const PairState& S = st[b];
   const int n = ASYNC ? n_async : S.n_src;
   const GridDesc& g = gd[ASYNC ? g_async : (grid_of ? grid_of[b] : b)];
@@ -320,10 +362,12 @@
       const bool live = lane < m && (PCAQ || KD || B.weight != VOX_DEAD);
       if constexpr (FAST) {
         float u[3] = {(xt0 - B.mh[0]) - B.ml[0], (xt1 - B.mh[1]) - B.ml[1], (xt2 - B.mh[2]) - B.ml[2]};
-        eval_hit_fast<PCA, decltype(mid)>(u, r, B.c, sc.d1f, sc.d2f, sc.kq, B.w, live, acc, mid);
+        if constexpr (SO) { mid(); eval_score_fast<PCA>(u, B.c, sc.d1f, sc.d2f, sc.kq, B.w, live, acc[0]); }
+        else eval_hit_fast<PCA, decltype(mid)>(u, r, B.c, sc.d1f, sc.d2f, sc.kq, B.w, live, acc, mid);
       } else {
         float u[3] = {(float)((double)xt0 - B.m0), (float)((double)xt1 - B.m1), (float)((double)xt2 - B.m2)};
-        eval_hit<PCA, decltype(mid), KD, ORD>(u, r, B.C, sc.d1, sc.d2f, B.w, live, acc, exp_tab, mid);
+        if constexpr (SO) { mid(); eval_score<PCA, ORD>(u, B.C, sc.d1, sc.d2f, B.w, live, acc[0], exp_tab); }
+        else eval_hit<PCA, decltype(mid), KD, ORD>(u, r, B.C, sc.d1, sc.d2f, B.w, live, acc, exp_tab, mid);
       }
       nhits += PCAQ ? (unsigned)m : (unsigned)__popcll(__ballot(live));
       qhead = (qhead + m) & (Q_CAP - 1);
@@ -463,6 +507,14 @@
       if (qcount > 0) drain(qcount);
       TL_STAMP(5);
     }
+    if constexpr (SO) {
+      const double v = score_tree((double)acc[0]);
+      if (lane == 0) {
+        gu64* PG = (gu64*)reinterpret_cast<unsigned long long*>(partials + ((size_t)b * rows_per_pair + rem) * NACC);
+        __hip_atomic_store(PG, (unsigned long long)__double_as_longlong(v), RLX_AGENT);
+        __hip_atomic_store(PG + 43, (unsigned long long)__double_as_longlong((double)nhits), RLX_AGENT);
+      }
+    } else {
     typedef unsigned int u2v __attribute__((ext_vector_type(2)));
     double accd[43];
     if constexpr (FAST) fast_acc_to_row(acc, accd);
@@ -502,6 +554,7 @@
         if (lane == 0) P[43] = (double)nhits;
       }
     }
+    }
     if (FINE) {
       __syncthreads();
       if (wv == 0 && lane < NACC)
@@ -515,7 +568,7 @@
   }
 }
 
-template <bool PCA, int ORD, int NROWS>
+template <bool PCA, int ORD, int NROWS, bool SO = false>
 __device__ __forceinline__ void sweep_rows_d1(const int b, const int rem0, const float* __restrict__ src, const size_t pitch,
                                               const GridDesc* __restrict__ gd, const BitWord* __restrict__ words, const VoxelRec* __restrict__ recs,
                                               double* partials, const int rows_per_pair, const SweepConst& sc, const double* exp_tab,
@@ -527,8 +580,8 @@
   constexpr int TP = 2, IT = 8, NST = IT / TP, Q_CAP = 512;
   const int lane = threadIdx.x & 63, wv = threadIdx.x >> 6;
   const unsigned long long lt_mask = (1ull << lane) - 1ull;
-  __shared__ unsigned q_ent[WAVES][Q_CAP];
-  __shared__ float stage[WAVES][64 * IT][6];
+  auto& q_ent = item_lds<unsigned[WAVES][Q_CAP], 4>();
+  auto& stage = item_lds<float[WAVES][64 * IT][6], 5>();
   const GridDesc& g = gd[g_idx];
   const float* X = src + (size_t)b * 3 * pitch;
   const BitWord* W = words + g.word_off;
@@ -569,7 +622,8 @@
     float r[3] = {sp[3], sp[4], sp[5]};
     const bool live = lane < m && B.weight != VOX_DEAD;
     float u[3] = {(float)((double)xt0 - B.m0), (float)((double)xt1 - B.m1), (float)((double)xt2 - B.m2)};
-    eval_hit<PCA, decltype(mid), false, ORD>(u, r, B.C, sc.d1, sc.d2f, PCA ? (double)B.weight : 1.0, live, acc, exp_tab, mid);
+    if constexpr (SO) { mid(); eval_score<PCA, ORD>(u, B.C, sc.d1, sc.d2f, PCA ? (double)B.weight : 1.0, live, acc[0], exp_tab); }
+    else eval_hit<PCA, decltype(mid), false, ORD>(u, r, B.C, sc.d1, sc.d2f, PCA ? (double)B.weight : 1.0, live, acc, exp_tab, mid);
     nhits += (unsigned)__popcll(__ballot(live));
     qhead = (qhead + m) & (Q_CAP - 1);
     qcount -= m;
@@ -659,6 +713,14 @@
     if (qcount > 0) { Batch Bt; fetch(0, qcount, Bt); eval_batch(Bt, qcount, NoHook()); }
     TL_STAMP(5);
     if (s + 1 < S_TOTAL) { probe(s + 1); load_points(s + 2); }
+    if constexpr (SO) {
+      const double v = score_tree(acc[0]);
+      if (lane == 0) {
+        gu64* PG = (gu64*)reinterpret_cast<unsigned long long*>(partials + ((size_t)b * rows_per_pair + rem0 + s / NST) * NACC);
+        __hip_atomic_store(PG, (unsigned long long)__double_as_longlong(v), RLX_AGENT);
+        __hip_atomic_store(PG + 43, (unsigned long long)__double_as_longlong((double)nhits), RLX_AGENT);
+      }
+    } else {
     typedef unsigned int u2v __attribute__((ext_vector_type(2)));
     double P1[22], P2[11];
 #pragma unroll
@@ -684,6 +746,7 @@
 #pragma unroll
       for (int i = 0; i < 11; i++) if (rb + i < 43) __hip_atomic_store(PG + rb + i, (unsigned long long)__double_as_longlong(P2[i]), RLX_AGENT);
       if (lane == 0) __hip_atomic_store(PG + 43, (unsigned long long)__double_as_longlong((double)nhits), RLX_AGENT);
+    }
     }
 #pragma unroll
     for (int a = 0; a < 43; a++) acc[a] = 0.0;
diff --git a/lv_slam_amd/csrc/ndt_types.hpp b/lv_slam_amd/csrc/ndt_types.hpp
--- a/lv_slam_amd/csrc/ndt_types.hpp
+++ b/lv_slam_amd/csrc/ndt_types.hpp
@@ -57,6 +57,7 @@
 struct PairState {
   float  T[12];
   float  Rj[9];
+  int    last_sweep;
   double p[6];
   double dir[6];
   double a_t;
@@ -72,6 +73,8 @@
   float  reb_inc[16];
   long long reb_tag;
 };
+
+static_assert(offsetof(PairState, last_sweep) == 84 && offsetof(PairState, p) == 88, "last_sweep sits in the padding behind the pose words");
 
 struct SweepConst {
   double d1;
diff --git a/lv_slam_amd/csrc/ndt_update.hpp b/lv_slam_amd/csrc/ndt_update.hpp
--- a/lv_slam_amd/csrc/ndt_update.hpp
+++ b/lv_slam_amd/csrc/ndt_update.hpp
@@ -50,7 +50,7 @@
   ndtm::se3_log(ndtm::se3_from_Rt(R, t), S.p);
   float Tdummy[12];
   ndtm::pose_to_f32(S.p, Tdummy, S.Rj);
-  S.it = 0; S.phase = PH_SWEEP0; S.converged = 0; S.sweeps = 1; S.a_t = 0; S.hits = 0; S.score = 0; S.mt_loops = 0;
+  S.it = 0; S.phase = PH_SWEEP0; S.converged = 0; S.sweeps = 1; S.a_t = 0; S.hits = 0; S.score = 0; S.mt_loops = 0; S.last_sweep = 0;
   for (int a = 0; a < 16; a++) S.inc_cm[a] = S.prev_inc_cm[a] = (a % 5 == 0) ? 1.f : 0.f;
   S.n_src = n_src;
   S.grid_status = grid_status;
@@ -72,7 +72,7 @@
   active_list[0] = b; ctl->n_active = 1;
   for (int r = 0; r < 3; r++) for (int c = 0; c < 4; c++) S.T[r * 4 + c] = T_cm[c * 4 + r];
   for (int a = 0; a < 9; a++) S.Rj[a] = Rj[a];
-  S.phase = PH_SWEEP0; S.n_src = src_cnt[b]; S.grid_status = gd[b].status; S.it = 0; S.sweeps = 1;
+  S.phase = PH_SWEEP0; S.n_src = src_cnt[b]; S.grid_status = gd[b].status; S.it = 0; S.sweeps = 1; S.last_sweep = 0;
 }
 NDT_KERNEL void k_set_pose_p(PairState* st, int b, const double* __restrict__ p, const int* __restrict__ src_cnt, const GridDesc* __restrict__ gd,
                              int* active_list, SweepCtl* ctl, int for_hessian) {
@@ -81,7 +81,7 @@
   double pp[6];
   for (int a = 0; a < 6; a++) { pp[a] = p[a]; S.xt[a] = p[a]; }
   ndtm::pose_to_f32(pp, S.T, S.Rj);
-  S.phase = for_hessian ? PH_HESS : PH_SWEEP0; S.n_src = src_cnt[b]; S.grid_status = gd[b].status; S.it = 0; S.sweeps = 1;
+  S.phase = for_hessian ? PH_HESS : PH_SWEEP0; S.n_src = src_cnt[b]; S.grid_status = gd[b].status; S.it = 0; S.sweeps = 1; S.last_sweep = 0;
 }
 
 __device__ inline double mt_cmin(double a, double b) { return b < a ? b : a; }
@@ -275,7 +275,8 @@
 
 __device__ __forceinline__ int newton_update(PairState& S, mi355ndt_result* res, double step_max, double eps, int max_iterations, int mt,
                                              volatile double* sol = nullptr ,
-                                             const bool rebased = false ) {
+                                             const bool rebased = false ,
+                                             const bool score_only_last = false) {
   const int lane = threadIdx.x & 63;
   ndtm::SE3 e_dp, e_p;
   const bool pre = (mt == 0) && (S.phase == PH_STEP) && !rebased;
@@ -330,6 +331,9 @@
     }
     for (int a = 0; a < 6; a++) S.p[a] = pn[a];
     const bool conv = (S.it > max_iterations) || (S.it && (fabs(S.a_t) < eps));
+#ifdef NDT_DEBUG_LAST_SWEEP
+    if (S.last_sweep && !conv) printf("newton_update: last_sweep set for a step that does not end the pair (it %d, a_t %g)\n", S.it, S.a_t);
+#endif
     S.it++;
     if (conv) { finalize_pair(S, res, 1); return NEWTON_DONE; }
   }
@@ -368,6 +372,7 @@
     double xt[6];
     for (int a = 0; a < 6; a++) { S.dir[a] = d[a]; xt[a] = S.p[a] + d[a] * a_t; S.xt[a] = xt[a]; }
     S.a_t = a_t;
+    S.last_sweep = (mt == 0 && score_only_last && ((S.it > max_iterations) || (S.it && (fabs(a_t) < eps)))) ? 1 : 0;
     S.phi0 = -S.score;
     S.dphi0 = dphi0 >= 0 ? -dphi0 : dphi0;
     ndtm::pose_to_f32(xt, S.T, S.Rj);
diff --git a/lv_slam_amd/ndt.py b/lv_slam_amd/ndt.py
--- a/lv_slam_amd/ndt.py
+++ b/lv_slam_amd/ndt.py
@@ -45,7 +45,7 @@
                 ("update_launches", C.c_longlong), ("async_fallbacks", C.c_longlong), ("stream_launches", C.c_longlong),
                 ("stream_carried", C.c_longlong), ("stream_redone", C.c_longlong), ("cloud_uploads", C.c_longlong), ("cloud_upload_bytes", C.c_longlong),
                 ("cloud_transfers", C.c_longlong), ("cloud_promotions", C.c_longlong),
-                ("stream_reserved_slots", C.c_longlong), ("stream_launch_slots", C.c_longlong)]
+                ("stream_reserved_slots", C.c_longlong), ("stream_launch_slots", C.c_longlong), ("score_only_sweeps", C.c_longlong)]
 
 
 class SeqParams(C.Structure):
@@ -83,6 +83,7 @@
 WARN_TOLERANCE_ARITH = 1
 OPT_ARITH = 7
 OPT_F32_SUM_ORDER = 1
+OPT_SCORE_ONLY_LAST_SWEEP = 8
 
 _LIB = None
 
```
